# jaeyong-song/network_distributed_pytorch

Hardware: AMD Instinct MI355X
Metric: samples/sec + bytes/step all-reduced, ResNet18 CIFAR10 PowerSGD r=4, 1/2/4/8 GPU (higher is better)
Workload: dtype fp32; 1 GPU; model=resnet18, num_classes=1000, global_batch=512, per_gpu_batch=512, parallelism=dp1, reducer=powersgd, powersgd_rank=4, overlap=False, link_emulation=none, channels_last=False, stock_model_ops=False, hip_graph=full, tuned_gemms=True

## Files before the change

network_distributed_pytorch_amd/csrc/bindings.cpp:

```cpp
#include <algorithm>
#include <ATen/hip/HIPContext.h>
#include <torch/extension.h>

#include <cstring>

#include "ndp_kernels.h"
#include "plan.h"

namespace {

using ndp::MatGeom;
using ndp::MatPtrs;
using ndp::PItem;
using ndp::QItem;
using ndp::SegEntry;
using ndp::UItem;

hipStream_t cur_stream() { return at::hip::getCurrentHIPStream().stream(); }

void check_launch(const char* what) {
  const hipError_t err = hipGetLastError();
  TORCH_CHECK(err == hipSuccess, what, ": ", hipGetErrorString(err));
}

// ... 1060 lines not shown
  const int64_t M = g.size(0);
  const int N = (int)g.size(1);
  const int chunks = ndp::colsum_chunks(M, N);
  float* dp = deferred_part(part_out, (int64_t)chunks * N, "gelu_bwd_colsum");
  torch::Tensor part;
  if (dp == nullptr) part = torch::empty({(int64_t)chunks * N}, g.options());
  ndp::launch_gelu_bwd_colsum(g.data_ptr<float>(), h.data_ptr<float>(), dh.data_ptr<float>(), M, N,
                              dp ? dp : part.data_ptr<float>(), dp ? nullptr : db.data_ptr<float>(), cur_stream());
  check_launch("launch_gelu_bwd_colsum");
  return dp ? chunks : 0;
}

void ce_fwd(torch::Tensor x, torch::Tensor tgt, torch::Tensor dl, torch::Tensor scratch, torch::Tensor loss,
            torch::Tensor ctr, int64_t ignore_index, c10::optional<torch::Tensor> acc) {
  check_f32(x, "logits"); check_f32(dl, "dl"); check_f32(scratch, "scratch"); check_f32(loss, "loss");
  float* ap = nullptr;
  if (acc.has_value()) {
    check_f32(*acc, "acc");
    TORCH_CHECK(acc->numel() == 1, "ce_fwd: acc must be a one-element fp32 tensor");
    ap = acc->data_ptr<float>();
  }
  check_dev(tgt, "target"); check_dev(ctr, "ctr");
  TORCH_CHECK(x.dim() == 2 && x.is_contiguous() && dl.sizes() == x.sizes() && dl.is_contiguous(),
              "ce_fwd: logits / dl must be contiguous [B, K]");
  TORCH_CHECK(tgt.scalar_type() == torch::kInt64 && tgt.is_contiguous() && tgt.numel() == x.size(0),
              "ce_fwd: target must be contiguous int64 [B]");
  TORCH_CHECK(scratch.numel() >= x.size(0) + 1 && loss.numel() == 1, "ce_fwd: scratch / loss size");
  TORCH_CHECK(ctr.scalar_type() == torch::kInt32 && ctr.numel() >= 1, "ce_fwd: int32 counter");
  TORCH_CHECK(x.size(0) >= 1 && x.size(0) < (1LL << 31) && x.size(1) >= 1, "ce_fwd: empty batch");
  const int B = (int)x.size(0);
  float* sp = scratch.data_ptr<float>();
  ndp::launch_ce_fwd(x.data_ptr<float>(), tgt.data_ptr<int64_t>(), B, (int)x.size(1), ignore_index,
                     dl.data_ptr<float>(), sp, loss.data_ptr<float>(), sp + B,
                     reinterpret_cast<unsigned*>(ctr.data_ptr<int32_t>()), cur_stream(), ap);
  check_launch("launch_ce_fwd");
}

void ce_bwd(torch::Tensor dl, torch::Tensor g, torch::Tensor scratch, torch::Tensor dx) {
  check_f32(dl, "dl"); check_f32(g, "grad"); check_f32(scratch, "scratch"); check_f32(dx, "dx");
  TORCH_CHECK(dl.is_contiguous() && dx.is_contiguous() && dx.sizes() == dl.sizes() && dl.dim() == 2, "ce_bwd: shapes");
  TORCH_CHECK(g.numel() == 1 && scratch.numel() >= dl.size(0) + 1, "ce_bwd: scalar grad / scratch");
  TORCH_CHECK((reinterpret_cast<uintptr_t>(dl.data_ptr()) & 15) == 0 && (reinterpret_cast<uintptr_t>(dx.data_ptr()) & 15) == 0,
              "ce_bwd: 16-B aligned tensors");
  ndp::launch_ce_bwd(dl.data_ptr<float>(), g.data_ptr<float>(), scratch.data_ptr<float>() + dl.size(0),
                     dx.data_ptr<float>(), dl.numel(), cur_stream());
  check_launch("launch_ce_bwd");
}

static ndp::LnDrop ln_drop(int64_t mode, double p, const c10::optional<torch::Tensor>& seed,
                           const c10::optional<torch::Tensor>& da, int64_t numel) {
  ndp::LnDrop d{nullptr, 0u, 1.f, 0, nullptr};
  if (mode == 0 || p <= 0.0) return d;
  TORCH_CHECK(mode == 1 || mode == 2, "ln: dropout mode 0 / 1 / 2");
  TORCH_CHECK(p < 1.0, "ln: dropout p < 1");
  TORCH_CHECK(seed.has_value() && seed->is_cuda() && seed->scalar_type() == torch::kInt32 && seed->numel() >= 1,
              "ln: dropout needs a device int32 seed");
  d.seed = seed->data_ptr<int32_t>();
  const double t = p * 4294967296.0;
  d.thr = t >= 4294967295.0 ? 0xFFFFFFFFu : (uint32_t)t;
  d.scale = (float)(1.0 / (1.0 - p));
  d.mode = (int)mode;
  if (da.has_value()) {
    check_f32(*da, "da");
    TORCH_CHECK(da->is_contiguous() && da->numel() == numel, "ln: da [R, D]");
    d.da = da->data_ptr<float>();
  }
  return d;
}

void ln_fwd(torch::Tensor a, c10::optional<torch::Tensor> b, torch::Tensor gamma, torch::Tensor beta, torch::Tensor y,
            torch::Tensor s, torch::Tensor mean, torch::Tensor rstd, double eps, int64_t drop_mode, double p,
            c10::optional<torch::Tensor> seed) {
  check_f32(a, "a"); check_f32(gamma, "gamma"); check_f32(beta, "beta"); check_f32(y, "y"); check_f32(s, "s");
  check_f32(mean, "mean"); check_f32(rstd, "rstd");
  const int D = (int)a.size(-1);
  TORCH_CHECK(ndp::ln_supported(D) && gamma.numel() == D && beta.numel() == D, "ln_fwd: unsupported D");
  const int64_t R = a.numel() / D;
  for (auto* t : {&a, &y, &s}) TORCH_CHECK(t->is_contiguous() && t->numel() == R * D, "ln_fwd: contiguous [R, D]");
  if (b.has_value()) {
    check_f32(*b, "b");
    TORCH_CHECK(b->is_contiguous() && b->sizes() == a.sizes(), "ln_fwd: residual shape");
  }
  TORCH_CHECK(mean.numel() == R && rstd.numel() == R, "ln_fwd: stats size");
  ndp::launch_ln_fwd(a.data_ptr<float>(), opt_f32(b, "b"), gamma.data_ptr<float>(), beta.data_ptr<float>(),
                     y.data_ptr<float>(), s.data_ptr<float>(), mean.data_ptr<float>(), rstd.data_ptr<float>(), R, D,
                     (float)eps, cur_stream(), ln_drop(drop_mode, p, seed, c10::nullopt, R * D));
  check_launch("launch_ln_fwd");
}

int64_t ln_bwd(torch::Tensor dy, torch::Tensor s, torch::Tensor mean, torch::Tensor rstd, torch::Tensor gamma,
               torch::Tensor dx, torch::Tensor dgb, int64_t drop_mode, double p, c10::optional<torch::Tensor> seed,
               c10::optional<torch::Tensor> da, c10::optional<torch::Tensor> part_out) {
  check_f32(dy, "dy"); check_f32(s, "s"); check_f32(mean, "mean"); check_f32(rstd, "rstd"); check_f32(gamma, "gamma");
  check_f32(dx, "dx"); check_f32(dgb, "dgb");
  const int D = (int)s.size(-1);
  const int64_t R = s.numel() / D;
  TORCH_CHECK(ndp::ln_supported(D) && gamma.numel() == D && dgb.numel() == 2 * D, "ln_bwd: unsupported D");
  for (auto* t : {&dy, &s, &dx}) TORCH_CHECK(t->is_contiguous() && t->numel() == R * D, "ln_bwd: contiguous [R, D]");
  const ndp::LnDrop dp = ln_drop(drop_mode, p, seed, da, R * D);
  TORCH_CHECK(dp.mode != 1 || dp.da != nullptr, "ln_bwd: input dropout needs da");
  const int wgs = ndp::ln_bwd_wgs(R);
  float* pp = deferred_part(part_out, (int64_t)wgs * 2 * D, "ln_bwd");
  torch::Tensor part;
  if (pp == nullptr) part = torch::empty({(int64_t)wgs * 2 * D}, s.options());
  ndp::launch_ln_bwd(dy.data_ptr<float>(), s.data_ptr<float>(), mean.data_ptr<float>(), rstd.data_ptr<float>(),
                     gamma.data_ptr<float>(), dx.data_ptr<float>(), pp ? pp : part.data_ptr<float>(),
                     pp ? nullptr : dgb.data_ptr<float>(), R, D, cur_stream(), dp);
  check_launch("launch_ln_bwd");
  return pp ? wgs : 0;
}

void embedding_backward(torch::Tensor ids, torch::Tensor gout, torch::Tensor gw, int64_t pad, torch::Tensor perm,
                        torch::Tensor row_start, torch::Tensor row_cnt) {
  check_dev(ids, "ids"); check_f32(gout, "grad_out"); check_f32(gw, "grad_weight");
  check_dev(perm, "perm"); check_dev(row_start, "row_start"); check_dev(row_cnt, "row_cnt");
  TORCH_CHECK(ids.scalar_type() == torch::kInt64 && ids.is_contiguous(), "embedding_backward: ids must be contiguous int64");
  TORCH_CHECK(gw.dim() == 2 && gw.size(1) % 4 == 0, "embedding_backward: grad_weight [V, D] with D % 4 == 0");
  const int64_t T = ids.numel(), V = gw.size(0), D = gw.size(1);
  TORCH_CHECK(gout.numel() == T * D, "embedding_backward: grad_out must be [T, D]");
  TORCH_CHECK((reinterpret_cast<uintptr_t>(gout.data_ptr()) & 15) == 0 && (reinterpret_cast<uintptr_t>(gw.data_ptr()) & 15) == 0,
              "embedding_backward: 16-B aligned grad tensors");
  for (auto* t : {&perm, &row_start, &row_cnt})
    TORCH_CHECK(t->scalar_type() == torch::kInt32 && t->is_contiguous(), "embedding_backward: int32 scratch");
  TORCH_CHECK(perm.numel() >= T && row_start.numel() >= V && row_cnt.numel() >= V, "embedding_backward: scratch too small");
  TORCH_CHECK(T < (1LL << 29) && V < (1LL << 31), "embedding_backward: too many tokens / rows");
  ndp::launch_embedding_backward(ids.data_ptr<int64_t>(), (int)T, gout.data_ptr<float>(), (int)V, (int)D, (int)pad,
                                 perm.data_ptr<int32_t>(), row_start.data_ptr<int32_t>(), row_cnt.data_ptr<int32_t>(),
                                 gw.data_ptr<float>(), cur_stream());
  check_launch("launch_embedding_backward");
}

void attn_check(const torch::Tensor& t, const char* n, const torch::Tensor& q) {
  check_f32(t, n);
  TORCH_CHECK(t.sizes() == q.sizes() && t.is_contiguous(), n, ": contiguous [B, S, H, 64] like q");
}

int64_t attn_ld(const torch::Tensor& t, const char* n, const torch::Tensor& q) {
  TORCH_CHECK(t.is_cuda(), n, " must be a device (HIP) tensor");
  TORCH_CHECK(t.scalar_type() == torch::kFloat32 && t.sizes() == q.sizes(), n, ": fp32 [B, S, H, 64] like q");
  const int64_t S = t.size(1), H = t.size(2), ld = t.stride(1);
  TORCH_CHECK(t.stride(3) == 1 && t.stride(2) == 64 && t.stride(0) == S * ld && ld >= H * 64 && ld % 4 == 0 &&
                  (reinterpret_cast<uintptr_t>(t.data_ptr()) & 15) == 0,
              n, ": needs [B, S, H, 64] rows with a 16-B aligned token stride");
  return ld;
}

const int32_t* attn_seed(const c10::optional<torch::Tensor>& seed, double p_drop) {
  TORCH_CHECK(p_drop >= 0.0 && p_drop < 1.0, "attn: p_drop in [0, 1)");
  if (p_drop == 0.0) return nullptr;
  TORCH_CHECK(seed.has_value(), "attn: dropout needs a device seed tensor");
  check_dev(*seed, "seed");
  TORCH_CHECK(seed->scalar_type() == torch::kInt32 && seed->numel() >= 1, "attn: seed must be int32[1]");
  return seed->data_ptr<int32_t>();
}

void attn_fwd(torch::Tensor q, torch::Tensor k, torch::Tensor v, c10::optional<torch::Tensor> mask, torch::Tensor o,
              torch::Tensor lse, double scale, c10::optional<torch::Tensor> seed, double p_drop) {
  TORCH_CHECK(q.dim() == 4 && q.size(3) == 64, "attn: q must be [B, S, H, 64]");
  const int64_t ld = attn_ld(q, "q", q);
  TORCH_CHECK(attn_ld(k, "k", q) == ld && attn_ld(v, "v", q) == ld, "attn: q / k / v need one token stride");
  attn_check(o, "o", q); check_f32(lse, "lse");
  const int B = (int)q.size(0), S = (int)q.size(1), H = (int)q.size(2);
  TORCH_CHECK(lse.numel() >= 2 * (int64_t)B * H * S, "attn: lse must hold 2*B*H*S floats");
  const int32_t* mp = nullptr;
  if (mask.has_value()) {
    check_dev(*mask, "mask");
    TORCH_CHECK(mask->scalar_type() == torch::kInt32 && mask->is_contiguous() && mask->numel() == (int64_t)B * S,
                "attn: mask must be int32 [B, S]");
    mp = mask->data_ptr<int32_t>();
  }
  const int32_t* sp = attn_seed(seed, p_drop);
  ndp::launch_attn_fwd(q.data_ptr<float>(), k.data_ptr<float>(), v.data_ptr<float>(), mp, o.data_ptr<float>(),
                       lse.data_ptr<float>(), B, S, H, (float)scale, sp, (float)p_drop, cur_stream(), ld);
  check_launch("launch_attn_fwd");
}

void attn_bwd(torch::Tensor q, torch::Tensor k, torch::Tensor v, c10::optional<torch::Tensor> mask, torch::Tensor o,
              torch::Tensor dout, torch::Tensor lse, torch::Tensor delta, torch::Tensor dq, torch::Tensor dk,
              torch::Tensor dv, double scale, c10::optional<torch::Tensor> seed, double p_drop) {
  TORCH_CHECK(q.dim() == 4 && q.size(3) == 64, "attn: q must be [B, S, H, 64]");
  const int64_t ld = attn_ld(q, "q", q);
  for (auto* t : {&k, &v, &dq, &dk, &dv})
    TORCH_CHECK(attn_ld(*t, "q/k/v grads", q) == ld, "attn: q / k / v and their grads need one token stride");
  attn_check(o, "o", q); attn_check(dout, "dout", q);
  check_f32(lse, "lse"); check_f32(delta, "delta");
  const int B = (int)q.size(0), S = (int)q.size(1), H = (int)q.size(2);
  TORCH_CHECK(lse.numel() >= 2 * (int64_t)B * H * S && delta.numel() >= (int64_t)B * H * S,
              "attn: lse/delta too small");
  const int32_t* mp = nullptr;
  if (mask.has_value()) {
    check_dev(*mask, "mask");
    TORCH_CHECK(mask->scalar_type() == torch::kInt32 && mask->is_contiguous() && mask->numel() == (int64_t)B * S,
                "attn: mask must be int32 [B, S]");
    mp = mask->data_ptr<int32_t>();
  }
  const int32_t* sp = attn_seed(seed, p_drop);
  ndp::launch_attn_bwd(q.data_ptr<float>(), k.data_ptr<float>(), v.data_ptr<float>(), mp, o.data_ptr<float>(),
                       dout.data_ptr<float>(), lse.data_ptr<float>(), delta.data_ptr<float>(), dq.data_ptr<float>(),
                       dk.data_ptr<float>(), dv.data_ptr<float>(), B, S, H, (float)scale, sp,
                       (float)p_drop, cur_stream(), ld);
  check_launch("launch_attn_bwd");
}

}

void register_comm(py::module& m);
namespace ndp {
void* ipc_new(int rank, int nranks, int device, int64_t capacity_bytes);
void ipc_delete(void* c);
std::string ipc_handle(void* c);
void ipc_open(void* c, const std::vector<std::string>& h);
void ipc_all_reduce_many(void* c, const std::vector<at::Tensor>& ts, const std::string& op, int64_t stream);
int64_t ipc_error(void* c);
void ipc_check(void* c);
void ipc_destroy(void* c);
std::string ipc_bus_id(void* c);
int64_t ipc_info(void* c, int what);
}

struct IpcCommPy {
  void* c;
  IpcCommPy(int rank, int nranks, int device, int64_t cap) : c(ndp::ipc_new(rank, nranks, device, cap)) {}
  ~IpcCommPy() { ndp::ipc_delete(c); }
};

void register_ipc(py::module& m) {
  py::class_<IpcCommPy, std::shared_ptr<IpcCommPy>>(m, "IpcComm")
      .def(py::init<int, int, int, int64_t>(), py::arg("rank"), py::arg("nranks"), py::arg("device"),
           py::arg("capacity_bytes") = 8 << 20)
      .def("handle", [](IpcCommPy& s) { return py::bytes(ndp::ipc_handle(s.c)); })
      .def("open", [](IpcCommPy& s, const std::vector<std::string>& h) { ndp::ipc_open(s.c, h); })
      .def("all_reduce", [](IpcCommPy& s, torch::Tensor t, const std::string& op, int64_t stream) {
            ndp::ipc_all_reduce_many(s.c, {t}, op, stream);
          }, py::arg("t"), py::arg("op") = "sum", py::arg("stream") = 0)
      .def("all_reduce_many", [](IpcCommPy& s, const std::vector<torch::Tensor>& ts, const std::string& op,
                                 int64_t stream) { ndp::ipc_all_reduce_many(s.c, ts, op, stream); },
           py::arg("ts"), py::arg("op") = "sum", py::arg("stream") = 0)
      .def("error", [](IpcCommPy& s) { return ndp::ipc_error(s.c); })
      .def("check", [](IpcCommPy& s) { ndp::ipc_check(s.c); })
      .def("destroy", [](IpcCommPy& s) { ndp::ipc_destroy(s.c); })
      .def("bus_id", [](IpcCommPy& s) { return ndp::ipc_bus_id(s.c); })
      .def_property_readonly("rank", [](IpcCommPy& s) { return ndp::ipc_info(s.c, 0); })
      .def_property_readonly("nranks", [](IpcCommPy& s) { return ndp::ipc_info(s.c, 1); })
      .def_property_readonly("device", [](IpcCommPy& s) { return ndp::ipc_info(s.c, 2); })
      .def_property_readonly("capacity", [](IpcCommPy& s) { return ndp::ipc_info(s.c, 3); })
      .def_property_readonly("alive", [](IpcCommPy& s) { return ndp::ipc_info(s.c, 4) != 0; })
      .def_property_readonly("uncached", [](IpcCommPy& s) { return ndp::ipc_info(s.c, 5) != 0; })
      .def_property_readonly("launches", [](IpcCommPy& s) { return ndp::ipc_info(s.c, 6); });
}

PYBIND11_MODULE(TORCH_EXTENSION_NAME, m) {
  m.doc() = "network_distributed_pytorch_amd native gfx950 kernels + plan builder";
  m.attr("SIZEOF_MATGEOM") = (int)sizeof(MatGeom);
  m.attr("SIZEOF_MATPTRS") = (int)sizeof(MatPtrs);
  m.attr("SIZEOF_SEGENTRY") = (int)sizeof(SegEntry);
  m.attr("MAX_RANK") = ndp::kMaxRank;
  m.def("build_plan", &build_plan, "Build the PowerSGD execution plan (host)");
  m.def("patch_geom_vec", &patch_geom_vec);
  m.def("make_mat_ptrs", &make_mat_ptrs);
  m.def("make_seg_table", &make_seg_table);
  m.def("make_orth_geom", &make_orth_geom);
  m.def("psgd_p", &psgd_p, py::arg("geom"), py::arg("ptrs"), py::arg("items"), py::arg("q_warm"), py::arg("p_part"),
        py::arg("fuse_ef"), py::arg("max_rank"), py::arg("p_prev") = OptT(), py::arg("p_out") = OptT(),
        py::arg("p_ctr") = OptT(), py::arg("seg_entries") = OptT(), py::arg("seg_prefix") = OptT(),
        py::arg("seg_n") = 0, py::arg("seg_blocks") = 0, py::arg("p_cols") = (int64_t)ndp::kPKW);
  m.def("psgd_q", &psgd_q, py::arg("geom"), py::arg("ptrs"), py::arg("items"), py::arg("p_hat"), py::arg("q_part"),
        py::arg("max_rank"), py::arg("q_out") = OptT(), py::arg("q_ctr") = OptT(), py::arg("q_fin_max") = 1 << 30);
  m.def("psgd_orth", &psgd_orth, py::arg("geom"), py::arg("items"), py::arg("p"), py::arg("p_div"),
        py::arg("eps"), py::arg("max_rank"), py::arg("scratch"), py::arg("ctr"), py::arg("n_items_total") = -1,
        py::arg("max_spins") = -1);
  m.def("orth_coresident_cap", &ndp::orth_coresident_cap);
  m.def("psgd_update", &psgd_update, py::arg("geom"), py::arg("ptrs"), py::arg("items"), py::arg("p_hat"),
        py::arg("q_sum"), py::arg("q_div"), py::arg("q_warm"), py::arg("mode"), py::arg("lr"), py::arg("momentum"),
        py::arg("max_rank"), py::arg("p_prev") = c10::optional<torch::Tensor>(), py::arg("r1_buf") = OptT(),
        py::arg("r1_div") = 1.0, py::arg("r1_mom") = OptT(), py::arg("r1_x") = OptT(), py::arg("r1_g") = OptT());
  m.def("rank1_step", &rank1_step);
  m.def("seg_reduce", &seg_reduce);
  m.def("sgd_momentum", &sgd_momentum);
  m.def("add", &add);
  m.def("delay_ns", &delay_ns);
  m.def("bn_fwd", &bn_fwd, py::arg("x"), py::arg("res"), py::arg("y"), py::arg("gamma"), py::arg("beta"),
        py::arg("rmean"), py::arg("rvar"), py::arg("nbt"), py::arg("save_mean"), py::arg("save_invstd"),
        py::arg("part"), py::arg("eps"), py::arg("momentum"), py::arg("relu"), py::arg("training"),
        py::arg("single"), py::arg("xpart") = py::none(), py::arg("nslab") = 0, py::arg("xstats") = py::none(),
        py::arg("xS") = 0);
  m.def("bn_bwd", &bn_bwd, py::arg("dy"), py::arg("y"), py::arg("x"), py::arg("gamma"), py::arg("save_mean"),
        py::arg("save_invstd"), py::arg("dx"), py::arg("dres"), py::arg("dgamma"), py::arg("dbeta"), py::arg("part"),
        py::arg("relu"), py::arg("single"), py::arg("dypart") = py::none(), py::arg("nslab") = 0,
        py::arg("dyadd") = py::none(), py::arg("mbeta") = py::none(), py::arg("dstats") = py::none(),
        py::arg("dS") = 0);
  m.def("bn_relu_maxpool", &bn_relu_maxpool, py::arg("x"), py::arg("y"), py::arg("idx"), py::arg("gamma"),
        py::arg("beta"), py::arg("rmean"), py::arg("rvar"), py::arg("nbt"), py::arg("save_mean"),
        py::arg("save_invstd"), py::arg("part"), py::arg("eps"), py::arg("momentum"), py::arg("xstats") = py::none(),
        py::arg("xS") = 0);
  m.def("bn_two_kernel_path", [](int64_t N, int64_t C, int64_t HW, bool single) {
    return ndp::bn_two_kernel_path((int)N, (int)C, (int)HW, single ? 1 : 0);
  });
  m.def("bn_set_vec4", &ndp::bn_set_vec4);
  m.def("bn_pair_ok", &ndp::bn_pair_ok);
  m.def("bn_pair_fwd", &bn_pair_fwd);
  m.def("bn_pair_bwd", &bn_pair_bwd);
  m.def("wino_set_enabled", &ndp::wino_set_enabled);
  m.def("conv_set_stem_psplit", &ndp::conv_set_stem_psplit);
  m.def("bn_slices", &bn_slices);
  m.def("slab_sum", &slab_sum);
  m.def("bn_part_numel", &bn_part_numel);
  m.def("maxpool_fwd", &maxpool_fwd);
  m.def("maxpool_bwd", &maxpool_bwd);
  m.def("maxpool_bwd_bnstats", &maxpool_bwd_bnstats, py::arg("dy"), py::arg("idx"), py::arg("dx"), py::arg("x"),
        py::arg("gamma"), py::arg("beta"), py::arg("mean"), py::arg("invstd"), py::arg("stats"));
  m.def("stem_pool_bwd_apply", &stem_pool_bwd_apply);
  m.def("checksum", &checksum);
  m.def("flag_signal", &flag_signal);
  m.def("flag_wait", &flag_wait, py::arg("flags"), py::arg("i"), py::arg("seen"), py::arg("err"),
        py::arg("timeout_us"), py::arg("host_err") = c10::optional<torch::Tensor>());
  m.def("toeplitz_expand", &toeplitz_expand);
  m.def("toeplitz_fold", &toeplitz_fold);
  m.def("toeplitz_expand_many", &toeplitz_expand_many);
  m.def("toeplitz_fold_many", &toeplitz_fold_many);
  m.def("slab_sum_many", &slab_sum_many);
  m.def("gradw_finish", &gradw_finish, py::arg("slabs"), py::arg("folds"));
  m.def("conv_plan", &conv_plan, py::arg("geom"), py::arg("batch"));
  m.def("conv_fwd", &conv_fwd, py::arg("x"), py::arg("w"), py::arg("y"), py::arg("geom"), py::arg("part") = py::none(),
        py::arg("defer") = false, py::arg("stats") = py::none(), py::arg("wino_u") = py::none(),
        py::arg("pair") = false);
  m.def("conv_flush_pending_fwd", []() {
    ndp::conv_flush_pending_fwd();
    check_launch("conv_flush_pending_fwd");
  });
  m.def("wino_weights", &wino_weights);
  m.def("wino_weights_many", &wino_weights_many);
  m.def("conv_wino", [](const std::vector<int64_t>& geom, int64_t B, bool dgrad) {
    const ndp::ConvGeom g = conv_geom(geom);
    const int cls = ndp::conv_direct_class(g);
    return cls >= 0 && B > 0 && B % ndp::conv_fwd_imgs(cls) == 0 && ndp::conv_wino(cls, g, (int)B, dgrad);
  });
  m.def("conv_stats_slices", &conv_stats_slices, py::arg("geom"), py::arg("batch"));
  m.def("conv_dgrad", &conv_dgrad, py::arg("dy"), py::arg("w"), py::arg("dx"), py::arg("geom"),
        py::arg("part") = py::none(), py::arg("addend") = py::none(), py::arg("defer") = false,
        py::arg("stats") = py::none(), py::arg("bn_x") = py::none(), py::arg("bn_y") = py::none(),
        py::arg("bn_mean") = py::none(), py::arg("bn_invstd") = py::none(), py::arg("wino_u") = py::none());
  m.def("conv_dgrad_stats_slices", [](const std::vector<int64_t>& geom, int64_t B) -> int64_t {
    const ndp::ConvGeom g = conv_geom(geom);
    const int cls = ndp::conv_direct_class(g);
    if (cls < 0 || B <= 0 || B % ndp::conv_fwd_imgs(cls)) return 0;
    return ndp::conv_dgrad_stats_slices(cls, g, (int)B);
  }, py::arg("geom"), py::arg("batch"));
  m.def("conv_wgrad", &conv_wgrad, py::arg("x"), py::arg("dy"), py::arg("part"), py::arg("dw"), py::arg("geom"),
        py::arg("pair") = false);
  m.def("conv_flush_pending", []() {
    ndp::conv_flush_pending();
    check_launch("conv_flush_pending");
  });
  m.def("tg_plan", &tg_plan);
  m.def("tg_describe", &tg_describe);
  m.def("tg_fwd", &tg_fwd, py::arg("x"), py::arg("w"), py::arg("y"), py::arg("geom"), py::arg("part") = py::none(),
        py::arg("defer") = false);
  m.def("tg_dgrad", &tg_dgrad, py::arg("dy"), py::arg("w"), py::arg("dx"), py::arg("geom"),
        py::arg("part") = py::none(), py::arg("addend") = py::none(), py::arg("defer") = false);
  m.def("tg_wgrad", &tg_wgrad, py::arg("x"), py::arg("dy"), py::arg("out"), py::arg("geom"),
        py::arg("part") = py::none(), py::arg("defer") = false);
  m.def("embedding_backward", &embedding_backward);
  m.def("colsum", &colsum, py::arg("g"), py::arg("out"), py::arg("part") = c10::optional<torch::Tensor>());
  m.def("gelu_bwd_colsum", &gelu_bwd_colsum, py::arg("g"), py::arg("h"), py::arg("dh"), py::arg("db"),
        py::arg("part") = c10::optional<torch::Tensor>());
  m.def("ce_fwd", &ce_fwd, py::arg("x"), py::arg("tgt"), py::arg("dl"), py::arg("scratch"), py::arg("loss"),
        py::arg("ctr"), py::arg("ignore_index"), py::arg("acc") = py::none());
  m.def("ln_fwd", &ln_fwd, py::arg("a"), py::arg("b"), py::arg("gamma"), py::arg("beta"), py::arg("y"), py::arg("s"),
        py::arg("mean"), py::arg("rstd"), py::arg("eps"), py::arg("drop_mode") = 0, py::arg("p") = 0.0,
        py::arg("seed") = c10::optional<torch::Tensor>());
  m.def("ln_bwd", &ln_bwd, py::arg("dy"), py::arg("s"), py::arg("mean"), py::arg("rstd"), py::arg("gamma"),
        py::arg("dx"), py::arg("dgb"), py::arg("drop_mode") = 0, py::arg("p") = 0.0,
        py::arg("seed") = c10::optional<torch::Tensor>(), py::arg("da") = c10::optional<torch::Tensor>(),
        py::arg("part") = c10::optional<torch::Tensor>());
  m.def("ln_bwd_wgs", [](int64_t R) { return (int64_t)ndp::ln_bwd_wgs(R); });
  m.def("colsum_chunks", [](int64_t M, int64_t N) { return (int64_t)ndp::colsum_chunks(M, (int)N); });
  m.def("ce_bwd", &ce_bwd);
  m.def("attn_fwd", &attn_fwd);
  m.def("attn_bwd", &attn_bwd);
  register_comm(m);
  register_ipc(m);
}
```

network_distributed_pytorch_amd/csrc/conv.hip:

```cpp
#include <hip/hip_runtime.h>
#include <stdlib.h>

#include "ndp_kernels.h"
#include "wino_dpp.h"

namespace ndp {

typedef float f32x4e __attribute__((ext_vector_type(4)));

__global__ __launch_bounds__(256) void toeplitz_expand_kernel(const float* __restrict__ w, float* __restrict__ wt,
                                                              ConvGeom g) {
  const int K = g.C * g.H * g.W;
  const int kcol = blockIdx.x * 256 + threadIdx.x;
  if (kcol >= K) return;
  const int n = blockIdx.y;
  const int OHW = g.OH * g.OW;
  const int co = n / OHW, ohw = n - co * OHW;
  const int oh = ohw / g.OW, ow = ohw - oh * g.OW;
  const int HW = g.H * g.W;
  const int ci = kcol / HW, ihw = kcol - ci * HW;
  const int ih = ihw / g.W, iw = ihw - ih * g.W;
  const int kh = ih - oh * g.stride + g.pad, kw = iw - ow * g.stride + g.pad;
  float v = 0.f;
  if (kh >= 0 && kh < g.KH && kw >= 0 && kw < g.KW) v = w[((co * g.C + ci) * g.KH + kh) * g.KW + kw];
  wt[(int64_t)n * K + kcol] = v;
}

template <int H, int W>
__device__ __forceinline__ void expand_row(const float* __restrict__ w, float* __restrict__ row, const ConvGeom& g,
                                           int co, int oh, int ow) {
  const int h0 = oh * g.stride - g.pad, w0 = ow * g.stride - g.pad;
  for (int ci = threadIdx.x; ci < g.C; ci += 256) {
    const float* wc = w + ((int64_t)co * g.C + ci) * g.KH * g.KW;
    float v[H * W];
#pragma unroll
    for (int ih = 0; ih < H; ++ih)
#pragma unroll
      for (int iw = 0; iw < W; ++iw) {
        const int kh = ih - h0, kw = iw - w0;
        v[ih * W + iw] = (kh >= 0 && kh < g.KH && kw >= 0 && kw < g.KW) ? wc[kh * g.KW + kw] : 0.f;
      }
    float* d = row + (int64_t)ci * (H * W);
    if constexpr ((H * W) % 4 == 0) {
#pragma unroll
      for (int j = 0; j < H * W; j += 4)
        *reinterpret_cast<f32x4e*>(d + j) = f32x4e{v[j], v[j + 1], v[j + 2], v[j + 3]};
    } else {
#pragma unroll
      for (int j = 0; j < H * W; ++j) d[j] = v[j];
    }
  }
}

__global__ __launch_bounds__(256) void toeplitz_expand_many_kernel(ExpandBatch b) {
  const int64_t r = blockIdx.x;
  int e = 0;
  while (e + 1 < b.n && r >= b.end[e]) ++e;
  const ConvGeom& g = b.g[e];
  const int n = (int)(r - (e ? b.end[e - 1] : 0));
  const int OHW = g.OH * g.OW;
  const int co = n / OHW, ohw = n - co * OHW;
  const int oh = ohw / g.OW, ow = ohw - oh * g.OW;
  float* row = b.wt[e] + (int64_t)n * g.C * g.H * g.W;
  if (g.H == 1 && g.W == 1) expand_row<1, 1>(b.w[e], row, g, co, oh, ow);
  else if (g.H == 2 && g.W == 2) expand_row<2, 2>(b.w[e], row, g, co, oh, ow);
  else if (g.H == 4 && g.W == 4) expand_row<4, 4>(b.w[e], row, g, co, oh, ow);
  else {
    const int K = g.C * g.H * g.W, HW = g.H * g.W;
    for (int kcol = threadIdx.x; kcol < K; kcol += 256) {
      const int ci = kcol / HW, ihw = kcol - ci * HW;
      const int ih = ihw / g.W, iw = ihw - ih * g.W;
      const int kh = ih - oh * g.stride + g.pad, kw = iw - ow * g.stride + g.pad;
      float v = 0.f;
      if (kh >= 0 && kh < g.KH && kw >= 0 && kw < g.KW) v = b.w[e][((co * g.C + ci) * g.KH + kh) * g.KW + kw];
      row[kcol] = v;
    }
  }
}

constexpr int kExpandRows = 8;
template <int H, int W>
__device__ __forceinline__ void expand_rows(const float* __restrict__ w, float* __restrict__ wt, const ConvGeom& g,
                                            int n0) {
  const int C = g.C, OHW = g.OH * g.OW;
  const int64_t K = (int64_t)C * H * W;
  for (int idx = threadIdx.x; idx < kExpandRows * C; idx += 256) {
    const int rr = idx / C, ci = idx - rr * C;
    const int n = n0 + rr;
    const int co = n / OHW, ohw = n - co * OHW;
    const int oh = ohw / g.OW, ow = ohw - oh * g.OW;
    const int h0 = oh * g.stride - g.pad, w0 = ow * g.stride - g.pad;
    const float* wc = w + ((int64_t)co * C + ci) * g.KH * g.KW;
    float v[H * W];
#pragma unroll
    for (int ih = 0; ih < H; ++ih)
#pragma unroll
      for (int iw = 0; iw < W; ++iw) {
        const int kh = ih - h0, kw = iw - w0;
        v[ih * W + iw] = (kh >= 0 && kh < g.KH && kw >= 0 && kw < g.KW) ? wc[kh * g.KW + kw] : 0.f;
      }
    float* d = wt + (int64_t)n * K + (int64_t)ci * (H * W);
    if constexpr ((H * W) % 4 == 0) {
#pragma unroll
      for (int j = 0; j < H * W; j += 4)
        *reinterpret_cast<f32x4e*>(d + j) = f32x4e{v[j], v[j + 1], v[j + 2], v[j + 3]};
    } else {
#pragma unroll
      for (int j = 0; j < H * W; ++j) d[j] = v[j];
    }
  }
}

__global__ __launch_bounds__(256) void toeplitz_expand_rows_kernel(ExpandBatch b) {
  const int64_t r0 = (int64_t)blockIdx.x * kExpandRows;
  int e = 0;
  while (e + 1 < b.n && r0 >= b.end[e]) ++e;
  const ConvGeom& g = b.g[e];
  const int n0 = (int)(r0 - (e ? b.end[e - 1] : 0));
  if (g.H == 1 && g.W == 1) expand_rows<1, 1>(b.w[e], b.wt[e], g, n0);
  else if (g.H == 2 && g.W == 2) expand_rows<2, 2>(b.w[e], b.wt[e], g, n0);
  else expand_rows<4, 4>(b.w[e], b.wt[e], g, n0);
}

void launch_toeplitz_expand_many(const ExpandBatch& b, hipStream_t s) {
  if (b.n <= 0) return;
  bool rows_ok = true;
  for (int e = 0; e < b.n; ++e) {
    const ConvGeom& g = b.g[e];
    const int64_t rows = b.end[e] - (e ? b.end[e - 1] : 0);
    rows_ok = rows_ok && rows % kExpandRows == 0 && g.H == g.W && (g.H == 1 || g.H == 2 || g.H == 4);
  }
  if (rows_ok)
    hipLaunchKernelGGL(toeplitz_expand_rows_kernel, dim3((unsigned)(b.end[b.n - 1] / kExpandRows)), dim3(256), 0, s,
                       b);
  else
    hipLaunchKernelGGL(toeplitz_expand_many_kernel, dim3((unsigned)b.end[b.n - 1]), dim3(256), 0, s, b);
}

constexpr int kFoldMaxTaps = 9;
__device__ __forceinline__ void fold_pair(const float* __restrict__ dwt, const ConvGeom& g, int pair,
                                          float (&acc)[kFoldMaxTaps]) {
  const int co = pair / g.C, ci = pair - co * g.C;
  const int K = g.C * g.H * g.W, HW = g.H * g.W;
#pragma unroll
  for (int t = 0; t < kFoldMaxTaps; ++t) acc[t] = 0.f;
  for (int oh = 0; oh < g.OH; ++oh)
    for (int ow = 0; ow < g.OW; ++ow) {
      const float* row = dwt + (int64_t)((co * g.OH + oh) * g.OW + ow) * K + ci * HW;
      for (int ih = 0; ih < g.H; ++ih) {
        const int kh = ih - oh * g.stride + g.pad;
        if (kh < 0 || kh >= g.KH) continue;
        for (int iw = 0; iw < g.W; ++iw) {
          const int kw = iw - ow * g.stride + g.pad;
          if (kw < 0 || kw >= g.KW) continue;
          const float v = row[ih * g.W + iw];
#pragma unroll
          for (int t = 0; t < kFoldMaxTaps; ++t)
            if (t == kh * g.KW + kw) acc[t] += v;
        }
      }
    }
}

template <int H, int W, int OH, int OW, int ST, int PD, int KH, int KW>
__device__ __forceinline__ void fold_pair_t(const float* __restrict__ dwt, int C, int pair,
                                            float (&acc)[kFoldMaxTaps]) {
  const int co = pair / C, ci = pair - co * C;
  const int64_t K = (int64_t)C * H * W;
#pragma unroll
  for (int t = 0; t < kFoldMaxTaps; ++t) acc[t] = 0.f;
  float v[OH * OW][H * W];
#pragma unroll
  for (int oh = 0; oh < OH; ++oh)
#pragma unroll
    for (int ow = 0; ow < OW; ++ow) {
      const float* row = dwt + (int64_t)((co * OH + oh) * OW + ow) * K + (int64_t)ci * (H * W);
#pragma unroll
      for (int ih = 0; ih < H; ++ih)
#pragma unroll
        for (int iw = 0; iw < W; ++iw) {
          const int kh = ih - oh * ST + PD, kw = iw - ow * ST + PD;
          v[oh * OW + ow][ih * W + iw] = (kh >= 0 && kh < KH && kw >= 0 && kw < KW) ? row[ih * W + iw] : 0.f;
        }
    }
#pragma unroll
  for (int oh = 0; oh < OH; ++oh)
#pragma unroll
    for (int ow = 0; ow < OW; ++ow)
#pragma unroll
      for (int ih = 0; ih < H; ++ih)
#pragma unroll
        for (int iw = 0; iw < W; ++iw) {
          const int kh = ih - oh * ST + PD, kw = iw - ow * ST + PD;
          if (kh >= 0 && kh < KH && kw >= 0 && kw < KW) acc[kh * KW + kw] += v[oh * OW + ow][ih * W + iw];
        }
}

__device__ __forceinline__ void fold_any(const float* __restrict__ dwt, const ConvGeom& g, int pair,
                                         float (&acc)[kFoldMaxTaps]) {
  const bool k3 = g.KH == 3 && g.KW == 3 && g.pad == 1, k1 = g.KH == 1 && g.KW == 1 && g.pad == 0;
  if (k3 && g.H == 2 && g.W == 2 && g.stride == 1) fold_pair_t<2, 2, 2, 2, 1, 1, 3, 3>(dwt, g.C, pair, acc);
  else if (k3 && g.H == 4 && g.W == 4 && g.stride == 2) fold_pair_t<4, 4, 2, 2, 2, 1, 3, 3>(dwt, g.C, pair, acc);
  else if (k1 && g.H == 4 && g.W == 4 && g.stride == 2) fold_pair_t<4, 4, 2, 2, 2, 0, 1, 1>(dwt, g.C, pair, acc);
  else if (k3 && g.H == 2 && g.W == 2 && g.stride == 2) fold_pair_t<2, 2, 1, 1, 2, 1, 3, 3>(dwt, g.C, pair, acc);
  else if (k1 && g.H == 2 && g.W == 2 && g.stride == 2) fold_pair_t<2, 2, 1, 1, 2, 0, 1, 1>(dwt, g.C, pair, acc);
  else if (k3 && g.H == 1 && g.W == 1 && g.stride == 1) fold_pair_t<1, 1, 1, 1, 1, 1, 3, 3>(dwt, g.C, pair, acc);
  else fold_pair(dwt, g, pair, acc);
}

__device__ __forceinline__ void fold_many_block(const FoldBatch& b, int64_t blk, float* __restrict__ stage) {
  const int64_t base = blk * 256;
  const int64_t i = base + threadIdx.x;
  const int64_t total = b.end[b.n - 1];
  int e = 0;
  while (e + 1 < b.n && base >= b.end[e]) ++e;
  const int64_t e_lo = e ? b.end[e - 1] : 0;
  const bool one_entry = base + 256 <= b.end[e];
  if (one_entry) {
    const ConvGeom& g = b.g[e];
    const int T = g.KH * g.KW;
    float acc[kFoldMaxTaps];
    fold_any(b.dwt[e], g, (int)(i - e_lo), acc);
#pragma unroll
    for (int t = 0; t < kFoldMaxTaps; ++t)
      if (t < T) stage[threadIdx.x * T + t] = acc[t];
    __syncthreads();
    float* out = b.dw[e] + (base - e_lo) * T;
    for (int k = threadIdx.x; k < 256 * T; k += 256) out[k] = stage[k];
    return;
  }
  if (i >= total) return;
  while (e + 1 < b.n && i >= b.end[e]) ++e;
  const ConvGeom& g = b.g[e];
  const int T = g.KH * g.KW;
  const int pair = (int)(i - (e ? b.end[e - 1] : 0));
  float acc[kFoldMaxTaps];
  fold_any(b.dwt[e], g, pair, acc);
  float* out = b.dw[e] + (int64_t)pair * T;
#pragma unroll
  for (int t = 0; t < kFoldMaxTaps; ++t)
    if (t < T) out[t] = acc[t];
}

__global__ __launch_bounds__(256) void toeplitz_fold_many_kernel(FoldBatch b) {
  __shared__ float stage[256 * kFoldMaxTaps];
  fold_many_block(b, blockIdx.x, stage);
}

void launch_toeplitz_fold_many(const FoldBatch& b, hipStream_t s) {
  if (b.n <= 0) return;
  const int64_t total = b.end[b.n - 1];
  hipLaunchKernelGGL(toeplitz_fold_many_kernel, dim3((unsigned)((total + 255) / 256)), dim3(256), 0, s, b);
}

void launch_toeplitz_expand(const float* w, float* wb, const ConvGeom& g, hipStream_t s) {
  const int N = g.Co * g.OH * g.OW, K = g.C * g.H * g.W;
  hipLaunchKernelGGL(toeplitz_expand_kernel, dim3((K + 255) / 256, N), dim3(256), 0, s, w, wb, g);
}

void launch_toeplitz_fold(const float* dwb, float* dw, const ConvGeom& g, hipStream_t s) {
  FoldBatch b{};
  b.dwt[0] = dwb;
  b.dw[0] = dw;
  b.g[0] = g;
  b.end[0] = (int64_t)g.Co * g.C;
  b.n = 1;
  launch_toeplitz_fold_many(b, s);
}



typedef float f32x16 __attribute__((ext_vector_type(16)));
typedef float f32x4c __attribute__((ext_vector_type(4)));

__device__ __forceinline__ f32x16 mfma32(float a, float b, f32x16 c) {
  return __builtin_amdgcn_mfma_f32_32x32x2f32(a, b, c, 0, 0, 0);
}

template <int R, int S, int ST, int PD, int H, int W, int CK, int BM, int IMGS, int WM, int NBUF, int KB, bool TRANSW,
          int PSPLIT = 1>
struct ConvFwdCfg {
  static constexpr int P = (H + 2 * PD - R) / ST + 1, Q = (W + 2 * PD - S) / ST + 1, PQ = P * Q;
  static_assert(PSPLIT == 1 || (IMGS == 1 && P % PSPLIT == 0), "row blocks of one image");
  static constexpr int LAYOUT = (ST == 1 && H == 8 && W == 8 && PD == 1 && IMGS == 1) ? 1
                                : (ST == 1 && H == 4 && W == 4 && IMGS % 2 == 0)      ? 2
                                : (ST == 2 && H == 8 && W == 8 && IMGS % 2 == 0)      ? 3
                                : (ST == 2 && H == 32 && W == 32 && R == 7 && IMGS == 1) ? 4
                                                                                       : 0;
  static constexpr bool DEINT = LAYOUT == 4;
  static constexpr int HALF = (W + 2 * PD + 2) / 2;
  static constexpr int Hp = H + 2 * PD;
  static constexpr int Wp = LAYOUT == 1 ? 12 : LAYOUT == 2 ? 8 : LAYOUT == 3 ? 12 : DEINT ? 2 * HALF : W + 2 * PD;
  __device__ static __forceinline__ constexpr int cpos(int col) {
    return DEINT ? (col & 1) * HALF + (col >> 1) : col;
  }
  static constexpr int HWp = (Hp * Wp) | 1, HW = H * W;
  static constexpr int IPAD0 = LAYOUT == 2 ? 4 : LAYOUT == 3 ? 1 : 0;
  static constexpr int IMGSTR = LAYOUT >= 2 ? (CK * HWp + 31) / 32 * 32 + IPAD0 : CK * HWp;
  static_assert(Wp >= W + 2 * PD && (!DEINT || (ST == 2 && HALF * 2 == Wp && (ST * Wp) % 32 == 16)),
                "row stride holds the zero border");
  __device__ static __forceinline__ void pix(int n, int& img, int& p, int& q) {
    if constexpr (LAYOUT == 1) {
      img = 0;
      p = (n & 31) >> 2;
// ... 145 lines not shown
      if (e < AE) {
        if (VEC) {
          if (!TRANSW) {
            const int r = e >> 2, k4 = r % (G::KK / 4), m = 4 * (r / (G::KK / 4)) + (e & 3);
            if constexpr (G::AV) {
              *reinterpret_cast<f32x4c*>(A + m * G::LDAM + 4 * k4) = ra[i];
            } else {
              float* d = A + 4 * k4 * G::LDA + m;
              d[0] = ra[i].x; d[G::LDA] = ra[i].y; d[2 * G::LDA] = ra[i].z; d[3 * G::LDA] = ra[i].w;
            }
          } else {
            const int c = e / (BM * G::RS / 4), f = 4 * (e - c * (BM * G::RS / 4));
#pragma unroll
            for (int j = 0; j < 4; ++j) {
              const int m = (f + j) / G::RS, rs = (f + j) - m * G::RS;
              const int kk = c * G::RS + (G::RS - 1 - rs);
              if constexpr (G::AV) A[m * G::LDAM + kk] = ra[i][j];
              else A[kk * G::LDA + m] = ra[i][j];
            }
          }
        } else {
#pragma unroll
          for (int j = 0; j < 4; ++j) {
            const int f = 4 * e + j, m = f / G::KK, kk = f - m * G::KK;
            if (f < BM * G::KK) {
              if constexpr (G::PAIRK) {
                const int row = G::pk_row(kk);
                if (row >= 0) A[row * G::LDA + m] = ra[i][j];
              } else if constexpr (G::AV) {
                A[m * G::LDAM + kk] = ra[i][j];
              } else {
                A[kk * G::LDA + m] = ra[i][j];
              }
            }
          }
        }
      }
    }
#pragma unroll
    for (int i = 0; i < BPT; ++i) {
      const int e = tid + 256 * i;
      if (e < B4I) {
        const int img = e / (CK * IHW / 4), rem = 4 * (e - img * (CK * IHW / 4));
        const int c = rem / IHW, hw = rem - c * IHW;
        const int hh = hw / IW, ww = hw - hh * IW;
        if constexpr (G::DEINT) {
          float* d = B + img * G::IMGSTR + c * G::HWp + (hh + PD) * G::Wp;
#pragma unroll
          for (int j = 0; j < 4; ++j) d[G::cpos(ww + PD + j)] = rb[i][j];
        } else {
          float* d = B + img * G::IMGSTR + c * G::HWp + (IUPS * hh + PD) * G::Wp + IUPS * ww + PD;
          d[0] = rb[i].x; d[IUPS] = rb[i].y; d[2 * IUPS] = rb[i].z; d[3 * IUPS] = rb[i].w;
        }
      }
    }
  };

  f32x16 acc[G::TM][G::TN];
#pragma unroll
  for (int tm = 0; tm < G::TM; ++tm)
#pragma unroll
    for (int tn = 0; tn < G::TN; ++tn)
#pragma unroll
      for (int r = 0; r < 16; ++r) acc[tm][tn][r] = 0.f;

  load(0);
  __syncthreads();
  store(0);
  __syncthreads();
  for (int ch = 0; ch < nchunks; ++ch) {
    const int cur = (NBUF == 2) ? (ch & 1) : 0;
    if (NBUF == 2 && ch + 1 < nchunks) load(ch + 1);
    const float* A = As + cur * G::A_SZ;
    const float* B = Bs + cur * G::B_SZ;
    float av[2][KB][G::TM], bv[2][KB][G::TN];
    auto fetch = [&](int blk, int slot) {
#pragma unroll
      for (int i = 0; i < KB; ++i) {
        const int t = blk * KB + i;
        int c = t / G::RS, rs = t - c * G::RS, r = rs / S, s = rs - r * S;
        if constexpr (G::PAIRK) {
          c = G::pk_c(t);
          r = G::pk_r(t);
          s = G::pk_s(t);
        }
        const int offb = c * G::HWp + r * G::Wp + (G::DEINT ? (s & 1) * G::HALF + (s >> 1) : s);
        if constexpr (!G::AV) {
#pragma unroll
          for (int tm = 0; tm < G::TM; ++tm) av[slot][i][tm] = A[a_base[tm] + t * G::LDA];
        }
#pragma unroll
        for (int tn = 0; tn < G::TN; ++tn) {
          if constexpr (G::PAIRK) bv[slot][i][tn] = B[(t < 56 ? b_base[tn] : b_base2[tn]) + offb];
          else bv[slot][i][tn] = B[b_base[tn] + offb];
        }
      }
      if constexpr (G::AV) {
#pragma unroll
        for (int tm = 0; tm < G::TM; ++tm)
#pragma unroll
          for (int q = 0; q < KB / 4; ++q) {
            const f32x4c v = *reinterpret_cast<const f32x4c*>(A + a_base[tm] + blk * KB + 4 * q);
#pragma unroll
            for (int j = 0; j < 4; ++j) av[slot][4 * q + j][tm] = v[j];
          }
      }
    };
    if constexpr (SCH == 1) __builtin_amdgcn_iglp_opt(0);
    fetch(0, 0);
#pragma unroll
    for (int blk = 0; blk < G::NBLK; ++blk) {
      if (blk + 1 < G::NBLK) fetch(blk + 1, (blk + 1) & 1);
#pragma unroll
      for (int i = 0; i < KB; ++i)
#pragma unroll
        for (int tm = 0; tm < G::TM; ++tm)
#pragma unroll
          for (int tn = 0; tn < G::TN; ++tn)
            acc[tm][tn] = mfma32(av[blk & 1][i][tm], bv[blk & 1][i][tn], acc[tm][tn]);
    }
    if constexpr (SCH == 2) {
#pragma unroll
      for (int i = 0; i < G::NSTEP * G::TM * G::TN; ++i) {
        __builtin_amdgcn_sched_group_barrier(0x008, 1, 0);
        __builtin_amdgcn_sched_group_barrier(0x100, 1, 0);
      }
    }
    if (ch + 1 < nchunks) {
      if (NBUF == 2) {
        store(cur ^ 1);
      } else {
        __syncthreads();
        load(ch + 1);
        store(0);
      }
    }
    __syncthreads();
  }

  if (gdim.z > 1) {
    float* pz = part + (int64_t)bid.z * slab;
#pragma unroll
    for (int tm = 0; tm < G::TM; ++tm)
#pragma unroll
      for (int tn = 0; tn < G::TN; ++tn) {
        const int n = (wn * G::TN + tn) * 32 + l32;
        int img, p, q;
        G::pix(n, img, p, q);
        p += prow0;
        float* pb = pz + (int64_t)(b0 + img) * Kout * G::PQ + p * G::Q + q;
#pragma unroll
        for (int r = 0; r < 16; ++r) {
          const int m = m0 + (wm * G::TM + tm) * 32 + (r & 3) + 8 * (r >> 2) + 4 * h;
          pb[(int64_t)m * G::PQ] = acc[tm][tn][r];
        }
      }
    return;
  }

  constexpr int OPQ = G::PQ * UPS * UPS;
  constexpr bool kStats = G::STATS_OK && UPS == 1;
  const bool stats = kStats && st.out != nullptr;
  const bool bstats = G::STATS2_OK && stats && st.bx != nullptr;
  float* L = smem;
  float* L2 = smem + BM * G::STATS_LDO;
#pragma unroll
  for (int tm = 0; tm < G::TM; ++tm)
#pragma unroll
    for (int tn = 0; tn < G::TN; ++tn) {
      const int n = (wn * G::TN + tn) * 32 + l32;
      int img, pp, qq;
      G::pix(n, img, pp, qq);
      pp += prow0;
      const int opix = UPS == 1 ? pp * G::Q + qq : pp * UPS * (UPS * G::Q) + qq * UPS;
      const int64_t yoff = (int64_t)(b0 + img) * Kout * OPQ + opix;
      float* yb = y + yoff;
      float ad[16], ad1[UPS == 2 ? 16 : 1], ad2[UPS == 2 ? 16 : 1], ad3[UPS == 2 ? 16 : 1];
      if (addend != nullptr) {
#pragma unroll
        for (int r = 0; r < 16; ++r) {
          const int m = m0 + (wm * G::TM + tm) * 32 + (r & 3) + 8 * (r >> 2) + 4 * h;
          const float* ap = addend + yoff + (int64_t)m * OPQ;
          ad[r] = ap[0];
          if constexpr (UPS == 2) {
            ad1[r] = ap[1];
            ad2[r] = ap[2 * G::Q];
            ad3[r] = ap[2 * G::Q + 1];
          }
        }
      } else {
#pragma unroll
        for (int r = 0; r < 16; ++r) {
          ad[r] = 0.f;
          if constexpr (UPS == 2) ad1[r] = ad2[r] = ad3[r] = 0.f;
        }
      }
      float bxv[16], byv[16], bmu[16], bis[16];
      if (kStats && bstats) {
#pragma unroll
        for (int r = 0; r < 16; ++r) {
          const int m = m0 + (wm * G::TM + tm) * 32 + (r & 3) + 8 * (r >> 2) + 4 * h;
          bxv[r] = st.bx[yoff + (int64_t)m * OPQ];
          byv[r] = st.by[yoff + (int64_t)m * OPQ];
          bmu[r] = st.mean[m];
          bis[r] = st.invstd[m];
        }
      }
#pragma unroll
      for (int r = 0; r < 16; ++r) {
        const int mloc = (wm * G::TM + tm) * 32 + (r & 3) + 8 * (r >> 2) + 4 * h;
        const int m = m0 + mloc;
        float* d = yb + (int64_t)m * OPQ;
        const float v = acc[tm][tn][r] + ad[r];
        d[0] = v;
        if constexpr (UPS == 2) {
          d[1] = ad1[r];
          d[2 * G::Q] = ad2[r];
          d[2 * G::Q + 1] = ad3[r];
        }
        if constexpr (kStats) {
          if (bstats) {
            const float dz = byv[r] > 0.f ? v : 0.f;
            L[mloc * G::STATS_LDO + n] = dz;
            L2[mloc * G::STATS_LDO + n] = dz * ((bxv[r] - bmu[r]) * bis[r]);
          } else if (stats) {
            L[mloc * G::STATS_LDO + n] = v;
          }
        }
      }
    }

  if constexpr (kStats) {
    if (stats) {
      __syncthreads();
      constexpr int TPC = G::STATS_TPC, NPT = G::BN / TPC;
      const int c = tid / TPC, j = tid - c * TPC;
      const float* src = L + c * G::STATS_LDO + j * NPT;
      const float* src2 = L2 + c * G::STATS_LDO + j * NPT;
      double sum = 0.0, sq = 0.0;
#pragma unroll 4
      for (int i = 0; i < NPT; i += 4) {
        const f32x4c v = *reinterpret_cast<const f32x4c*>(src + i);
        sum += (double)((v.x + v.y) + (v.z + v.w));
        if (bstats) {
          const f32x4c u = *reinterpret_cast<const f32x4c*>(src2 + i);
          sq += (double)((u.x + u.y) + (u.z + u.w));
        } else {
          sq += (double)((v.x * v.x + v.y * v.y) + (v.z * v.z + v.w * v.w));
        }
      }
#pragma unroll
      for (int o = 1; o < TPC; o <<= 1) {
        sum += __shfl_xor(sum, o, 64);
        sq += __shfl_xor(sq, o, 64);
      }
      if (j == 0) {
        double* d = st.out + ((int64_t)(m0 + c) * gdim.x + bid.x) * 2;
        d[0] = sum;
        d[1] = sq;
      }
    }
  }
}

template <int R, int S, int ST, int PD, int H, int W, int CK, int BM, int IMGS, int WM, int NBUF, int KB, bool TRANSW,
          bool VEC, int UPS = 1, int SCH = 0, int IUPS = 1, int PSPLIT = 1>
__global__ __launch_bounds__(256) void conv_fwd_kernel(const float* __restrict__ x, const float* __restrict__ w,
                                                       float* __restrict__ y, float* __restrict__ part, int Cin,
                                                       int Kout, int cps, int64_t slab,
                                                       const float* __restrict__ addend, ConvBnStats st) {
  extern __shared__ __attribute__((aligned(16))) float smem[];
  conv_fwd_body<R, S, ST, PD, H, W, CK, BM, IMGS, WM, NBUF, KB, TRANSW, VEC, UPS, SCH, IUPS, PSPLIT>(
      x, w, y, part, Cin, Kout, cps, slab, addend, st, make_uint3(blockIdx.x, blockIdx.y, blockIdx.z),
      make_uint3(gridDim.x, gridDim.y, gridDim.z), smem);
}

template <int R, int S, int ST, int PD, int H, int W, int CB, int BM, int NW, int NBPW, int KB>
struct ConvWgCfg {
  static constexpr int P = (H + 2 * PD - R) / ST + 1, Q = (W + 2 * PD - S) / ST + 1, PQ = P * Q;
  static constexpr int Hp = H + 2 * PD, Wp = W + 2 * PD, HWp = (Hp * Wp) | 1, HW = H * W;
  static constexpr int RS = R * S, J = CB * RS, JB = (J + 31) / 32, MB = BM / 32;
  static constexpr bool TAPMAJ = CB % 32 == 0;
  __device__ static __forceinline__ void col(int j, int& c, int& rs) {
    if constexpr (TAPMAJ) {
      rs = j / CB;
      c = j - rs * CB;
    } else {
      c = j / RS;
      rs = j - c * RS;
    }
  }
  static constexpr int NSTEP = PQ / 2, NBLK = NSTEP / KB;
  static constexpr bool AVW = KB % 4 == 0 && (PQ / 2) % 4 == 0;
  static constexpr int LDY = AVW ? PQ + (((PQ / 4) % 2 == 0) ? 4 : 8) : PQ + 1;
  static constexpr int A_SZ = BM * LDY;
  static constexpr int B_SZ = CB * HWp;
  static constexpr int NT = 64 * NW;
  static constexpr int A4 = BM * PQ / 4, B4 = CB * HW / 4;
  static constexpr int A_PER_T = (A4 + NT - 1) / NT, B_PER_T = (B4 + NT - 1) / NT;
  static constexpr int LDJ = J + 4;
  static constexpr size_t MAIN_BYTES = 2 * (size_t)(A_SZ + B_SZ) * sizeof(float);
  static constexpr size_t EPI_BYTES = TAPMAJ ? (size_t)BM * LDJ * sizeof(float) : 0;
  static constexpr size_t LDS_BYTES = MAIN_BYTES > EPI_BYTES ? MAIN_BYTES : EPI_BYTES;
  static_assert(MB * JB == NW * NBPW, "every wave owns NBPW 32x32 blocks");
  static_assert(P % 2 == 0 && PQ % 4 == 0 && HW % 4 == 0 && NSTEP % KB == 0, "pixel pairing / float4 loads");
};

template <int R, int S, int ST, int PD, int H, int W, int CB, int BM, int NW, int NBPW, int KB>
__device__ __forceinline__ void conv_wgrad_body(const float* __restrict__ x, const float* __restrict__ dy,
                                                float* __restrict__ part, int Cin, int Kout, int imgs_per_slice,
                                                const uint3 bid, float* __restrict__ smem) {
  using G = ConvWgCfg<R, S, ST, PD, H, W, CB, BM, NW, NBPW, KB>;
  float* As = smem;
  float* Bs = smem + 2 * G::A_SZ;
  const int tid = threadIdx.x, lane = tid & 63, wave = tid >> 6;
  const int h = lane >> 5, l32 = lane & 31;
  const int slice = bid.x, m0 = bid.y * BM, c0 = bid.z * CB;
  const int bb = slice * imgs_per_slice;

  for (int i = tid; i < 2 * G::B_SZ; i += G::NT) Bs[i] = 0.f;

  int a_base[NBPW], b_base[NBPW];
#pragma unroll
  for (int t = 0; t < NBPW; ++t) {
    const int blk = wave * NBPW + t;
    const int mb = blk / G::JB, jb = blk - mb * G::JB;
    const int j = jb * 32 + l32;
    a_base[t] = (mb * 32 + l32) * G::LDY + h * (G::PQ / 2);
    int c, rs;
    G::col(j, c, rs);
    const int r = rs / S, s = rs - r * S;
    b_base[t] = (j < G::J) ? c * G::HWp + r * G::Wp + s + h * (G::P / 2) * ST * G::Wp : 0;
  }

  f32x4c ra[G::A_PER_T], rb[G::B_PER_T];
  auto load = [&](int b) {
#pragma unroll
    for (int i = 0; i < G::A_PER_T; ++i) {
      const int e = tid + G::NT * i;
      f32x4c v = {0.f, 0.f, 0.f, 0.f};
      if (e < G::A4) v = *reinterpret_cast<const f32x4c*>(dy + ((int64_t)b * Kout + m0) * G::PQ + 4 * e);
      ra[i] = v;
    }
#pragma unroll
    for (int i = 0; i < G::B_PER_T; ++i) {
      const int e = tid + G::NT * i;
      f32x4c v = {0.f, 0.f, 0.f, 0.f};
      if (e < G::B4 && c0 + (4 * e) / G::HW < Cin)
        v = *reinterpret_cast<const f32x4c*>(x + ((int64_t)b * Cin + c0) * G::HW + 4 * e);
      rb[i] = v;
    }
  };
  auto store = [&](int buf) {
    float* A = As + buf * G::A_SZ;
    float* B = Bs + buf * G::B_SZ;
#pragma unroll
    for (int i = 0; i < G::A_PER_T; ++i) {
      const int e = tid + G::NT * i;
      if (e < G::A4) {
        const int m = (4 * e) / G::PQ, pq = 4 * e - m * G::PQ;
        float* d = A + m * G::LDY + pq;
        if constexpr (G::AVW) {
          *reinterpret_cast<f32x4c*>(d) = ra[i];
        } else {
          d[0] = ra[i].x; d[1] = ra[i].y; d[2] = ra[i].z; d[3] = ra[i].w;
        }
      }
    }
#pragma unroll
    for (int i = 0; i < G::B_PER_T; ++i) {
      const int e = tid + G::NT * i;
      if (e < G::B4) {
        const int c = (4 * e) / G::HW, hw = 4 * e - c * G::HW;
        const int hh = hw / W, ww = hw - hh * W;
        float* d = B + c * G::HWp + (hh + PD) * G::Wp + ww + PD;
        d[0] = rb[i].x; d[1] = rb[i].y; d[2] = rb[i].z; d[3] = rb[i].w;
      }
    }
  };

  f32x16 acc[NBPW];
#pragma unroll
  for (int t = 0; t < NBPW; ++t)
#pragma unroll
    for (int r = 0; r < 16; ++r) acc[t][r] = 0.f;

  load(bb);
  __syncthreads();
  store(0);
  __syncthreads();
  for (int i = 0; i < imgs_per_slice; ++i) {
    const int cur = i & 1;
    if (i + 1 < imgs_per_slice) load(bb + i + 1);
    const float* A = As + cur * G::A_SZ;
    const float* B = Bs + cur * G::B_SZ;
    float av[2][KB][NBPW], bv[2][KB][NBPW];
    auto fetch = [&](int blk, int slot) {
#pragma unroll
      for (int k = 0; k < KB; ++k) {
        const int t = blk * KB + k;
        const int p = t / G::Q, q = t - p * G::Q;
#pragma unroll
        for (int u = 0; u < NBPW; ++u) {
          if constexpr (!G::AVW) av[slot][k][u] = A[a_base[u] + t];
          bv[slot][k][u] = B[b_base[u] + p * ST * G::Wp + q * ST];
        }
      }
      if constexpr (G::AVW) {
#pragma unroll
        for (int u = 0; u < NBPW; ++u)
#pragma unroll
          for (int q4 = 0; q4 < KB / 4; ++q4) {
            const f32x4c v = *reinterpret_cast<const f32x4c*>(A + a_base[u] + blk * KB + 4 * q4);
#pragma unroll
            for (int j = 0; j < 4; ++j) av[slot][4 * q4 + j][u] = v[j];
          }
      }
    };
    fetch(0, 0);
#pragma unroll
    for (int blk = 0; blk < G::NBLK; ++blk) {
      if (blk + 1 < G::NBLK) fetch(blk + 1, (blk + 1) & 1);
#pragma unroll
      for (int k = 0; k < KB; ++k)
#pragma unroll
        for (int u = 0; u < NBPW; ++u) acc[u] = mfma32(av[blk & 1][k][u], bv[blk & 1][k][u], acc[u]);
    }
    if (i + 1 < imgs_per_slice) store(cur ^ 1);
    __syncthreads();
  }

  float* out = part + (int64_t)slice * Kout * Cin * G::RS;
  if constexpr (G::TAPMAJ && G::RS > 1) {
    float* st = smem;
#pragma unroll
    for (int t = 0; t < NBPW; ++t) {
      const int blk = wave * NBPW + t;
      const int mb = blk / G::JB, jb = blk - mb * G::JB;
      const int j = jb * 32 + l32;
      int c, rs;
      G::col(j, c, rs);
      if (j < G::J) {
#pragma unroll
        for (int r = 0; r < 16; ++r)
          st[(mb * 32 + (r & 3) + 8 * (r >> 2) + 4 * h) * G::LDJ + c * G::RS + rs] = acc[t][r];
      }
    }
    __syncthreads();
    const int lim = min(CB, Cin - c0) * G::RS;
    constexpr int J4 = G::J / 4;
    static_assert(G::J % 4 == 0, "float4 rows");
    for (int i = tid; i < BM * J4; i += G::NT) {
      const int mr = i / J4, q = 4 * (i - mr * J4);
      const f32x4c v = *reinterpret_cast<const f32x4c*>(st + mr * G::LDJ + q);
      float* o = out + ((int64_t)(m0 + mr) * Cin + c0) * G::RS + q;
      if (q + 3 < lim) {
        *reinterpret_cast<f32x4c*>(o) = v;
      } else {
#pragma unroll
        for (int k = 0; k < 4; ++k)
          if (q + k < lim) o[k] = v[k];
      }
    }
    return;
  }
#pragma unroll
  for (int t = 0; t < NBPW; ++t) {
    const int blk = wave * NBPW + t;
    const int mb = blk / G::JB, jb = blk - mb * G::JB;
    const int j = jb * 32 + l32;
    int c, rs;
    G::col(j, c, rs);
    if (j < G::J && c0 + c < Cin) {
#pragma unroll
      for (int r = 0; r < 16; ++r) {
        const int m = m0 + mb * 32 + (r & 3) + 8 * (r >> 2) + 4 * h;
        out[((int64_t)m * Cin + c0 + c) * G::RS + rs] = acc[t][r];
      }
    }
  }
}

template <int R, int S, int ST, int PD, int H, int W, int CB, int BM, int NW, int NBPW, int KB>
__global__ __launch_bounds__(64 * NW) void conv_wgrad_kernel(const float* __restrict__ x, const float* __restrict__ dy,
                                                             float* __restrict__ part, int Cin, int Kout,
                                                             int imgs_per_slice) {
  extern __shared__ __attribute__((aligned(16))) float smem[];
  conv_wgrad_body<R, S, ST, PD, H, W, CB, BM, NW, NBPW, KB>(x, dy, part, Cin, Kout, imgs_per_slice,
                                                           make_uint3(blockIdx.x, blockIdx.y, blockIdx.z), smem);
}

template <int WH, int IUPS, int R, int S, int ST, int PD, int H, int W, int CB, int BM, int NW, int NBPW, int KB>
__global__ __launch_bounds__(256, 2) void wino_direct_pair_kernel(WinoConvArgs A, uint3 ga, const float* __restrict__ x,
                                                                  const float* __restrict__ dy, float* __restrict__ part,
                                                                  int Cin, int Kout, int imgs, uint3 gw) {
  static_assert(NW <= 4, "grad-W workgroup within the pair's 256 threads");
  extern __shared__ __attribute__((aligned(16))) float smem[];
  const unsigned na = ga.x * ga.y * ga.z;
  unsigned b = blockIdx.x;
  if (b < na) {
    wino_dpp_body<WH, IUPS>(A, make_uint3(b % ga.x, (b / ga.x) % ga.y, b / (ga.x * ga.y)), ga, smem);
  } else {
    if (threadIdx.x >= 64 * NW) return;
    b -= na;
    conv_wgrad_body<R, S, ST, PD, H, W, CB, BM, NW, NBPW, KB>(
        x, dy, part, Cin, Kout, imgs, make_uint3(b % gw.x, (b / gw.x) % gw.y, b / (gw.x * gw.y)), smem);
  }
}

__global__ __launch_bounds__(256) void conv_slab_sum_kernel(const float* __restrict__ part, float* __restrict__ dw,
                                                            int64_t n, int n_slices,
                                                            const float* __restrict__ addend = nullptr) {
  __shared__ f32x4c red[16][16];
  const int col = threadIdx.x & 15, g = threadIdx.x >> 4;
  const int64_t i4 = ((int64_t)blockIdx.x * 16 + col) * 4;
  f32x4c acc = {0.f, 0.f, 0.f, 0.f};
  if (i4 < n) {
#pragma unroll 4
    for (int s = g; s < n_slices; s += 16) acc += *reinterpret_cast<const f32x4c*>(part + (int64_t)s * n + i4);
  }
  red[g][col] = acc;
  __syncthreads();
  if (g == 0 && i4 < n) {
    f32x4c t = red[0][col];
#pragma unroll
    for (int k = 1; k < 16; ++k) t += red[k][col];
    if (addend) t += *reinterpret_cast<const f32x4c*>(addend + i4);
    *reinterpret_cast<f32x4c*>(dw + i4) = t;
  }
}

__device__ __forceinline__ void slab_sum_many_block(const SlabBatch& b, int64_t blk, f32x4c (*red)[16]) {
  int e = 0;
  while (e + 1 < b.n && blk >= b.end[e]) ++e;
  const int64_t lb = blk - (e ? b.end[e - 1] : 0);
  const float* part = b.part[e];
  const int64_t n = b.numel[e];
  const int n_slices = b.slices[e];
  const int col = threadIdx.x & 15, g = threadIdx.x >> 4;
  const int64_t i4 = (lb * 16 + col) * 4;
  f32x4c acc = {0.f, 0.f, 0.f, 0.f};
  if (i4 < n) {
#pragma unroll 4
    for (int sl = g; sl < n_slices; sl += 16) {
      if (b.nt) acc += __builtin_nontemporal_load(reinterpret_cast<const f32x4c*>(part + (int64_t)sl * n + i4));
      else acc += *reinterpret_cast<const f32x4c*>(part + (int64_t)sl * n + i4);
    }
  }
  red[g][col] = acc;
  __syncthreads();
  if (g == 0 && i4 < n) {
    f32x4c t = red[0][col];
#pragma unroll
    for (int k = 1; k < 16; ++k) t += red[k][col];
    *reinterpret_cast<f32x4c*>(b.dw[e] + i4) = t;
  }
}

__global__ __launch_bounds__(256) void conv_slab_sum_many_kernel(SlabBatch b) {
  __shared__ f32x4c red[16][16];
  slab_sum_many_block(b, blockIdx.x, red);
}

__global__ __launch_bounds__(256) void gradw_finish_kernel(SlabBatch sb, FoldBatch fb) {
  constexpr int kFloats = 256 * kFoldMaxTaps > 16 * 16 * 4 ? 256 * kFoldMaxTaps : 16 * 16 * 4;
  __shared__ __attribute__((aligned(16))) float smem[kFloats];
  const int64_t n_slab = sb.n > 0 ? sb.end[sb.n - 1] : 0;
  const int64_t blk = blockIdx.x;
  if (blk < n_slab) slab_sum_many_block(sb, blk, reinterpret_cast<f32x4c (*)[16]>(smem));
  else fold_many_block(fb, blk - n_slab, smem);
}

void launch_gradw_finish(const SlabBatch& sb, const FoldBatch& fb, hipStream_t s) {
  if (sb.n <= 0) return launch_toeplitz_fold_many(fb, s);
  if (fb.n <= 0) return launch_slab_sum_many(sb, s);
  const_cast<SlabBatch&>(sb).nt = 1;
  const int64_t blocks = sb.end[sb.n - 1] + (fb.end[fb.n - 1] + 255) / 256;
  hipLaunchKernelGGL(gradw_finish_kernel, dim3((unsigned)blocks), dim3(256), 0, s, sb, fb);
}

void launch_slab_sum_many(const SlabBatch& b, hipStream_t s) {
  const_cast<SlabBatch&>(b).nt = 1;
  if (b.n <= 0) return;
  hipLaunchKernelGGL(conv_slab_sum_many_kernel, dim3((unsigned)b.end[b.n - 1]), dim3(256), 0, s, b);
}

template <int P, int Q>
__global__ __launch_bounds__(256) void conv_slab_sum_ups_kernel(const float* __restrict__ part, float* __restrict__ dx,
                                                                int64_t slab, int n_slices,
                                                                const float* __restrict__ addend) {
  constexpr int F4R = (2 * Q) / 4, F4P = 2 * P * F4R;
  static_assert((2 * Q) % 4 == 0, "float4 rows");
  const int64_t i4 = (int64_t)blockIdx.x * 256 + threadIdx.x;
  if (i4 * 4 >= slab * 4) return;
  const int64_t plane = i4 / F4P;
  const int r4 = (int)(i4 - plane * F4P);
  const int row = r4 / F4R, half = r4 - row * F4R;
  f32x4c v = {0.f, 0.f, 0.f, 0.f};
  if (addend != nullptr) v = *reinterpret_cast<const f32x4c*>(addend + i4 * 4);
  if ((row & 1) == 0) {
    const int p = row >> 1, q0 = half * 2;
    const float* src = part + plane * (P * Q) + p * Q + q0;
    float a = 0.f, b = 0.f;
    for (int z = 0; z < n_slices; ++z) {
      a += src[z * slab];
      b += src[z * slab + 1];
    }
    v.x += a;
    v.z += b;
  }
  *reinterpret_cast<f32x4c*>(dx + i4 * 4) = v;
}

template <typename KernelT>
static void set_lds(KernelT k, size_t bytes) {
  hipFuncSetAttribute(reinterpret_cast<const void*>(k), hipFuncAttributeMaxDynamicSharedMemorySize, (int)bytes);
}

struct DirectDgradArgs {
  const float* dy;
  const float* w;
  float* dx;
  float* part;
  int Cin, Kout, cps;
  int64_t slab;
  const float* addend;
};
template <int DH, int DW, int DBM, int DIMGS, int R, int S, int ST, int PD, int H, int W, int CB, int BM, int NW,
          int NBPW, int KB>
__global__ __launch_bounds__(256) void direct_pair_kernel(DirectDgradArgs A, uint3 ga, const float* __restrict__ x,
                                                          const float* __restrict__ dy, float* __restrict__ part,
                                                          int Cin, int Kout, int imgs, uint3 gw) {
  static_assert(NW <= 4, "grad-W workgroup within the pair's 256 threads");
  extern __shared__ __attribute__((aligned(16))) float smem[];
  const unsigned na = ga.x * ga.y * ga.z;
  unsigned b = blockIdx.x;
  if (b < na) {
    conv_fwd_body<1, 1, 1, 0, DH, DW, 8, DBM, DIMGS, 2, 2, 4, true, true, 2>(
        A.dy, A.w, A.dx, A.part, A.Cin, A.Kout, A.cps, A.slab, A.addend, ConvBnStats{},
        make_uint3(b % ga.x, (b / ga.x) % ga.y, b / (ga.x * ga.y)), ga, smem);
  } else {
    if (threadIdx.x >= 64 * NW) return;
    b -= na;
    conv_wgrad_body<R, S, ST, PD, H, W, CB, BM, NW, NBPW, KB>(
        x, dy, part, Cin, Kout, imgs, make_uint3(b % gw.x, (b / gw.x) % gw.y, b / (gw.x * gw.y)), smem);
  }
}

template <int R, int S, int ST, int PD, int H, int W, int CK, int BM, int IMGS, int WM, int NBUF, int KB, bool TRANSW,
          bool VEC, int UPS = 1, int SCH = 0, int IUPS = 1, int PSPLIT = 1>
static int run_fwd(const float* x, const float* w, float* y, int B, int Cin, int Kout, int ksplit, float* part,
                   hipStream_t s, const float* addend = nullptr, bool defer = false,
                   ConvBnStats stats = ConvBnStats{nullptr, nullptr, nullptr, nullptr, nullptr}) {
  using G = ConvFwdCfg<R, S, ST, PD, H, W, CK, BM, IMGS, WM, NBUF, KB, TRANSW, PSPLIT>;
  auto k = conv_fwd_kernel<R, S, ST, PD, H, W, CK, BM, IMGS, WM, NBUF, KB, TRANSW, VEC, UPS, SCH, IUPS, PSPLIT>;
  static bool attr = false;
  if (!attr) { set_lds(k, G::LDS_BYTES); attr = true; }
  const int nchunks = (Cin + CK - 1) / CK;
  if (ksplit < 1 || part == nullptr) ksplit = 1;
  const int cps = (nchunks + ksplit - 1) / ksplit;
  ksplit = (nchunks + cps - 1) / cps;
  const int64_t slab = (int64_t)B * Kout * G::PQ;
  if (!(G::STATS_OK && UPS == 1) || ksplit > 1 || (stats.bx != nullptr && !G::STATS2_OK)) stats.out = nullptr;
  hipLaunchKernelGGL(k, dim3(B / IMGS * PSPLIT, Kout / BM, ksplit), dim3(256), G::LDS_BYTES, s, x, w, y, part, Cin, Kout, cps,
                     slab, ksplit > 1 ? nullptr : addend, stats);
  if (ksplit > 1 && defer && UPS == 1) return ksplit;
  if (ksplit > 1) {
    if constexpr (UPS == 1)
      hipLaunchKernelGGL(conv_slab_sum_kernel, dim3((unsigned)((slab / 4 + 15) / 16)), dim3(256), 0, s, part, y, slab,
                         ksplit, addend);
    else
      hipLaunchKernelGGL((conv_slab_sum_ups_kernel<G::P, G::Q>), dim3((unsigned)((slab + 255) / 256)), dim3(256), 0, s,
                         part, y, slab, ksplit, addend);
  }
  return 1;
}

struct FwdPart {
  const float* x;
  const float* w;
  float* y;
  float* part;
  int Cin, Kout, cps;
  int64_t slab;
};
__global__ __launch_bounds__(256) void ds_fwd_pair_kernel(FwdPart a, uint3 ga, FwdPart b, uint3 gb) {
  extern __shared__ __attribute__((aligned(16))) float smem[];
  const unsigned na = ga.x * ga.y * ga.z;
  unsigned k = blockIdx.x;
  if (k < na) {
    conv_fwd_body<3, 3, 2, 1, 8, 8, 8, 64, 4, 2, 2, 4, false, true>(
        a.x, a.w, a.y, a.part, a.Cin, a.Kout, a.cps, a.slab, nullptr, ConvBnStats{},
        make_uint3(k % ga.x, (k / ga.x) % ga.y, k / (ga.x * ga.y)), ga, smem);
  } else {
    k -= na;
    conv_fwd_body<1, 1, 2, 0, 8, 8, 8, 64, 4, 2, 2, 4, false, true>(
        b.x, b.w, b.y, b.part, b.Cin, b.Kout, b.cps, b.slab, nullptr, ConvBnStats{},
        make_uint3(k % gb.x, (k / gb.x) % gb.y, k / (gb.x * gb.y)), gb, smem);
  }
}

template <typename G>
static FwdPart fwd_part(const float* x, const float* w, float* y, float* part, int B, int Cin, int Kout, int& ksplit) {
  const int nchunks = (Cin + 8 - 1) / 8;
  if (ksplit < 1 || part == nullptr) ksplit = 1;
  const int cps = (nchunks + ksplit - 1) / ksplit;
  ksplit = (nchunks + cps - 1) / cps;
  return FwdPart{x, w, y, part, Cin, Kout, cps, (int64_t)B * Kout * G::PQ};
}

void launch_slab_sum(const float* part, float* out, int64_t n, int nslab, hipStream_t s, const float* addend) {
  hipLaunchKernelGGL(conv_slab_sum_kernel, dim3((unsigned)((n / 4 + 15) / 16)), dim3(256), 0, s, part, out, n, nslab,
                     addend);
}

template <int R, int S, int ST, int PD, int H, int W, int CB, int BM, int NW, int NBPW, int KB>
static void run_wgrad(const float* x, const float* dy, float* part, float* dw, int B, int Cin, int Kout,
                      int imgs, hipStream_t s) {
  using G = ConvWgCfg<R, S, ST, PD, H, W, CB, BM, NW, NBPW, KB>;
  auto k = conv_wgrad_kernel<R, S, ST, PD, H, W, CB, BM, NW, NBPW, KB>;
  static bool attr = false;
  if (!attr) { set_lds(k, G::LDS_BYTES); attr = true; }
  const int slices = B / imgs;
  hipLaunchKernelGGL(k, dim3(slices, Kout / BM, (Cin + CB - 1) / CB), dim3(G::NT), G::LDS_BYTES, s, x, dy, part, Cin,
                     Kout, imgs);
  if (dw == nullptr) return;
  const int64_t n = (int64_t)Kout * Cin * G::RS;
  hipLaunchKernelGGL(conv_slab_sum_kernel, dim3((unsigned)((n / 4 + 15) / 16)), dim3(256), 0, s, part, dw, n, slices);
}

int conv_direct_class(const ConvGeom& g) {
  if (g.KH == 3 && g.KW == 3 && g.pad == 1 && g.stride == 1 && g.H == 8 && g.W == 8 && g.C % 64 == 0 && g.Co % 64 == 0)
    return 0;
  if (g.KH == 3 && g.KW == 3 && g.pad == 1 && g.stride == 1 && g.H == 4 && g.W == 4 && g.C % 64 == 0 && g.Co % 64 == 0)
    return 1;
  if (g.KH == 3 && g.KW == 3 && g.pad == 1 && g.stride == 2 && g.H == 8 && g.W == 8 && g.C % 64 == 0 && g.Co % 64 == 0)
    return 2;
  if (g.KH == 7 && g.KW == 7 && g.pad == 3 && g.stride == 2 && g.H == 32 && g.W == 32 && g.C == 3 && g.Co % 64 == 0)
    return 3;
  if (g.KH == 1 && g.KW == 1 && g.pad == 0 && g.stride == 2 && g.H == 8 && g.W == 8 && g.C % 64 == 0 && g.Co % 64 == 0)
    return 4;
  if (g.KH == 1 && g.KW == 1 && g.pad == 0 && g.stride == 2 && g.H == 4 && g.W == 4 && g.C % 64 == 0 && g.Co % 64 == 0)
    return 5;
  return -1;
}

int conv_fwd_imgs(int cls) { return (cls == 0 || cls == 3) ? 1 : cls == 5 ? 16 : 4; }

static constexpr int kFillWgs = 256;

static int pow2_floor(int v) {
  int p = 1;
  while (p * 2 <= v) p *= 2;
  return p;
}

int conv_wgrad_imgs(int cls, const ConvGeom& g, int B) {
  if (cls == 0 && g.H == 8 && g.C % 16 == 0 && g.Co % 16 == 0 && B <= 128 && B % 4 == 0) {
    const int per_slice = (g.Co / 16) * (g.C / 16);
    int d = 32;
    while (d > 4 && (B % d != 0 || (B / d) * per_slice < kFillWgs)) d /= 2;
    if (B % d == 0 && wino_wgrad_red(B, d)) return d;
  }
  if (cls == 0 && g.H == 8 && g.C % 16 == 0 && g.Co % 16 == 0 && B >= 256 && B % 16 == 0 && wino_wgrad_red(B, 16)) {
    return 16;
  }
  int def = cls == 0 ? 8 : cls == 1 ? (B >= 512 ? 32 : 16) : cls == 2 ? 16 : cls == 4 ? 8 : cls == 5 ? 16 : 4;
  const int cb = cls == 3 ? 3 : 32;
  const int per_slice = (g.Co / 32) * ((g.C + cb - 1) / cb);
  while (def > 1 && B % def != 0) def /= 2;
  while (def > 1 && (B / def) * per_slice < kFillWgs && B % (def / 2) == 0) def /= 2;
  return def;
}

static constexpr int kConvMaxSplit = 4;

int conv_ksplit(int cls, const ConvGeom& g, int B, bool dgrad) {
  if (cls < 0 || cls == 3) return 1;
  if (dgrad && (cls == 4 || cls == 5) && B >= 512) return 1;
  const int inC = dgrad ? g.Co : g.C, outC = dgrad ? g.C : g.Co;
  const int imgs = (dgrad && cls == 2) ? 1 : conv_fwd_imgs(cls);
  const int base = (B / imgs) * (outC / 64);
  const int nchunks = inC / 8;
  int ks = 1;
  while (ks * 2 <= nchunks && base * ks < kFillWgs && ks * 2 <= kConvMaxSplit) ks *= 2;
  return pow2_floor(ks);
}
static int wino_slabs(const float* part, float* out, int64_t n, int ks, bool defer, const float* addend,
                      hipStream_t s) {
  if (defer) return ks;
  hipLaunchKernelGGL(conv_slab_sum_kernel, dim3((unsigned)((n / 4 + 15) / 16)), dim3(256), 0, s, part, out, n, ks,
                     addend);
  return 1;
}

bool conv_wino(int cls, const ConvGeom& g, int B, bool dgrad) {
  if (dgrad)
    return (cls == 0 || cls == 1 || cls == 2) && wino_ok(g.Co, g.C, B, g.H, g.W, conv_ksplit(cls, g, B, true));
  return (cls == 0 || cls == 1) && wino_ok(g.C, g.Co, B, g.H, g.W, conv_ksplit(cls, g, B, false));
}

static int g_stem_psplit = 0;
void conv_set_stem_psplit(int p) { g_stem_psplit = (p == 1 || p == 2 || p == 4) ? p : 0; }
int stem_psplit(int B) {
  if (g_stem_psplit) return g_stem_psplit;
  return B >= 256 ? 1 : B >= 128 ? 2 : 4;
}

int conv_fwd_stats_slices(int cls, const ConvGeom& g, int B) {
  static_assert(ConvFwdCfg<3, 3, 1, 1, 8, 8, 8, 64, 1, 2, 2, 4, false>::STATS_OK &&
                    ConvFwdCfg<7, 7, 2, 3, 32, 32, 4, 64, 1, 2, 1, 7, false>::STATS_OK &&
                    ConvFwdCfg<7, 7, 2, 3, 32, 32, 4, 64, 1, 2, 1, 7, false, 2>::STATS_OK &&
                    ConvFwdCfg<7, 7, 2, 3, 32, 32, 4, 64, 1, 2, 1, 7, false, 4>::STATS_OK,
                "statistics epilogue fits every layer1 / stem tile");
  if (cls != 0 && cls != 3) return 0;
  if (conv_ksplit(cls, g, B, false) != 1) return 0;
  if (cls == 3) return B * stem_psplit(B);
  return conv_wino(cls, g, B, false) ? B / wino_imgs(g.H) : B / conv_fwd_imgs(cls);
}
int conv_dgrad_stats_slices(int cls, const ConvGeom& g, int B) {
  static_assert(ConvFwdCfg<3, 3, 1, 1, 8, 8, 8, 64, 1, 2, 2, 4, true>::STATS2_OK,
                "backward statistics epilogue fits the layer1 grad-x tiles");
  if ((cls != 0 && cls != 2) || conv_ksplit(cls, g, B, true) != 1) return 0;
  if (conv_wino(cls, g, B, true)) return B / wino_imgs(g.H);
  return cls == 2 ? B : B / conv_fwd_imgs(cls);
}
bool conv_dgrad_direct(int cls) { return cls >= 0 && cls <= 5 && cls != 3; }

namespace {
struct PendingFwd {
  const float* x = nullptr;
  const float* w = nullptr;
  float* y = nullptr;
  float* part = nullptr;
  int B = 0, ks = 1;
  bool defer = false;
  ConvGeom g{};
  hipStream_t s = nullptr;
};
PendingFwd g_pending_fwd;
using CfgC2 = ConvFwdCfg<3, 3, 2, 1, 8, 8, 8, 64, 4, 2, 2, 4, false, 1>;
using CfgC4 = ConvFwdCfg<1, 1, 2, 0, 8, 8, 8, 64, 4, 2, 2, 4, false, 1>;
}

void conv_flush_pending_fwd() {
  if (g_pending_fwd.x == nullptr) return;
  const PendingFwd p = g_pending_fwd;
  g_pending_fwd = PendingFwd{};
  run_fwd<1, 1, 2, 0, 8, 8, 8, 64, 4, 2, 2, 4, false, true>(p.x, p.w, p.y, p.B, p.g.C, p.g.Co, p.ks, p.part, p.s,
                                                           nullptr, p.defer);
}

int launch_conv_fwd(const float* x, const float* w, float* y, int B, const ConvGeom& g, float* part, hipStream_t s,
                    bool defer, double* stats_out, float* wino_u, bool pair) {
  const ConvBnStats stats{stats_out, nullptr, nullptr, nullptr, nullptr};
  const int cls = conv_direct_class(g);
  const int ks = conv_ksplit(cls, g, B, false);
  if (cls == 4 && pair && stats_out == nullptr) {
    conv_flush_pending_fwd();
    int k = ks;
    fwd_part<CfgC4>(x, w, y, part, B, g.C, g.Co, k);
    g_pending_fwd = PendingFwd{x, w, y, part, B, ks, defer, g, s};
    return (k > 1 && defer) ? k : 1;
  }
  if (cls == 2 && g_pending_fwd.x == x && g_pending_fwd.s == s && g_pending_fwd.B == B && stats_out == nullptr) {
    const PendingFwd p = g_pending_fwd;
    g_pending_fwd = PendingFwd{};
    int ka = ks, kb = p.ks;
    const FwdPart a = fwd_part<CfgC2>(x, w, y, part, B, g.C, g.Co, ka);
    const FwdPart b = fwd_part<CfgC4>(p.x, p.w, p.y, p.part, B, p.g.C, p.g.Co, kb);
    const uint3 ga = make_uint3((unsigned)(B / 4), (unsigned)(g.Co / 64), (unsigned)ka);
    const uint3 gb = make_uint3((unsigned)(B / 4), (unsigned)(p.g.Co / 64), (unsigned)kb);
    constexpr size_t lds = CfgC2::LDS_BYTES > CfgC4::LDS_BYTES ? CfgC2::LDS_BYTES : CfgC4::LDS_BYTES;
    static bool attr = false;
    if (!attr) { set_lds(ds_fwd_pair_kernel, lds); attr = true; }
    hipLaunchKernelGGL(ds_fwd_pair_kernel, dim3(ga.x * ga.y * ga.z + gb.x * gb.y * gb.z), dim3(256), lds, s, a, ga, b, gb);
    if (kb > 1 && !p.defer)
      hipLaunchKernelGGL(conv_slab_sum_kernel, dim3((unsigned)((b.slab / 4 + 15) / 16)), dim3(256), 0, s, p.part, p.y,
                         b.slab, kb, nullptr);
    if (ka > 1 && defer) return ka;
    if (ka > 1)
      hipLaunchKernelGGL(conv_slab_sum_kernel, dim3((unsigned)((a.slab / 4 + 15) / 16)), dim3(256), 0, s, part, y,
                         a.slab, ka, nullptr);
    return 1;
  }
  conv_flush_pending_fwd();
  if (wino_u != nullptr && conv_wino(cls, g, B, false)) {
    launch_wino_conv(x, wino_u, y, B, g.C, g.Co, g.H, false, 1, nullptr, ks > 1 ? ConvBnStats{} : stats, ks, part, s);
    return ks > 1 ? wino_slabs(part, y, (int64_t)B * g.Co * g.H * g.W, ks, defer, nullptr, s) : 1;
  }
  switch (cls) {
    case 0:
      return run_fwd<3, 3, 1, 1, 8, 8, 8, 64, 1, 2, 2, 4, false, true, 1, 2>(x, w, y, B, g.C, g.Co, ks, part, s,
                                                                             nullptr, defer, stats);
    case 1:
      return run_fwd<3, 3, 1, 1, 4, 4, 8, 64, 4, 2, 2, 4, false, true, 1, 2>(x, w, y, B, g.C, g.Co, ks, part, s,
                                                                             nullptr, defer);
    case 2:
      return run_fwd<3, 3, 2, 1, 8, 8, 8, 64, 4, 2, 2, 4, false, true>(x, w, y, B, g.C, g.Co, ks, part, s, nullptr,
                                                                       defer);
    case 3:
      switch (stem_psplit(B)) {
        case 4:
          return run_fwd<7, 7, 2, 3, 32, 32, 4, 64, 1, 2, 1, 7, false, false, 1, 0, 1, 4>(x, w, y, B, g.C, g.Co, 1, nullptr,
                                                                                        s, nullptr, false, stats);
        case 2:
          return run_fwd<7, 7, 2, 3, 32, 32, 4, 64, 1, 2, 1, 7, false, false, 1, 0, 1, 2>(x, w, y, B, g.C, g.Co, 1, nullptr,
                                                                                        s, nullptr, false, stats);
        default:
          return run_fwd<7, 7, 2, 3, 32, 32, 4, 64, 1, 2, 1, 7, false, false>(x, w, y, B, g.C, g.Co, 1, nullptr, s,
                                                                              nullptr, false, stats);
      }
    case 4:
      return run_fwd<1, 1, 2, 0, 8, 8, 8, 64, 4, 2, 2, 4, false, true>(x, w, y, B, g.C, g.Co, ks, part, s, nullptr,
                                                                       defer);
    case 5:
      return run_fwd<1, 1, 2, 0, 4, 4, 8, 64, 16, 2, 2, 4, false, true>(x, w, y, B, g.C, g.Co, ks, part, s, nullptr,
                                                                        defer);
    default: return 1;
  }
}

namespace {
struct PendingWgrad {
  const float* x = nullptr;
  const float* dy = nullptr;
  float* part = nullptr;
  int B = 0, imgs = 0, cls = -1;
  ConvGeom g{};
  hipStream_t s = nullptr;
};
constexpr int kPendingSlots = 2;
PendingWgrad g_pending[kPendingSlots];
unsigned g_pending_seq[kPendingSlots];
unsigned g_seq = 0;

void launch_pending(const PendingWgrad& p);
PendingWgrad* find_pending(const float* dy, int cls, int B, const ConvGeom& g, hipStream_t s) {
  for (auto& p : g_pending)
    if (p.dy == dy && p.cls == cls && p.s == s && p.B == B && p.g.C == g.C && p.g.Co == g.Co && p.g.H == g.H) return &p;
  return nullptr;
}
void flush_pending_dy(const float* dy) {
  for (auto& p : g_pending)
    if (p.dy == dy) {
      const PendingWgrad q = p;
      p = PendingWgrad{};
      launch_pending(q);
    }
}
void hold_pending(const PendingWgrad& q) {
  int k = -1;
  for (int i = 0; i < kPendingSlots; ++i)
    if (g_pending[i].dy == nullptr) { k = i; break; }
  if (k < 0) {
    k = g_pending_seq[0] <= g_pending_seq[1] ? 0 : 1;
    const PendingWgrad old = g_pending[k];
    g_pending[k] = PendingWgrad{};
    launch_pending(old);
  }
  g_pending[k] = q;
  g_pending_seq[k] = ++g_seq;
}

template <int WH, int IUPS, int R, int S, int ST, int PD, int H, int W, int CB, int BM, int NW, int NBPW, int KB>
void run_pair(const float* dy, const float* u, float* dx, int B, int inC, int outC, const float* addend,
              const ConvBnStats& st, int ks, float* part_x, const PendingWgrad& p, hipStream_t s) {
  using G = ConvWgCfg<R, S, ST, PD, H, W, CB, BM, NW, NBPW, KB>;
  auto k = wino_direct_pair_kernel<WH, IUPS, R, S, ST, PD, H, W, CB, BM, NW, NBPW, KB>;
  constexpr size_t lds = kWLds > G::LDS_BYTES ? kWLds : G::LDS_BYTES;
  static bool attr = false;
  if (!attr) { set_lds(k, lds); attr = true; }
  const WinoConvArgs a{dy, u + 16 * (int64_t)inC * outC,
                       dx, inC, outC, ks > 1 ? nullptr : addend, ks > 1 ? ConvBnStats{} : st, (inC / kWCK) / ks,
                       part_x, (int64_t)B * outC * WH * WH};
  const uint3 ga = make_uint3((unsigned)(B / wino_imgs(WH)), (unsigned)(outC / kWBM), (unsigned)ks);
  const uint3 gw = make_uint3((unsigned)(p.B / p.imgs), (unsigned)(p.g.Co / BM), (unsigned)((p.g.C + CB - 1) / CB));
  const unsigned n = ga.x * ga.y * ga.z + gw.x * gw.y * gw.z;
  hipLaunchKernelGGL(k, dim3(n), dim3(256), lds, s, a, ga, p.x, p.dy, p.part, p.g.C, p.g.Co, p.imgs, gw);
}
template <int DH, int DW, int DIMGS, int R, int S, int ST, int PD, int H, int W, int CB, int BM, int NW, int NBPW,
          int KB>
int run_direct_pair(const float* dy, const float* w, float* dx, int B, int Cin, int Kout, int ksplit, float* part,
                    const float* addend, const PendingWgrad& p, hipStream_t s) {
  using GF = ConvFwdCfg<1, 1, 1, 0, DH, DW, 8, 64, DIMGS, 2, 2, 4, true, 1>;
  using GW = ConvWgCfg<R, S, ST, PD, H, W, CB, BM, NW, NBPW, KB>;
  auto k = direct_pair_kernel<DH, DW, 64, DIMGS, R, S, ST, PD, H, W, CB, BM, NW, NBPW, KB>;
  constexpr size_t lds = GF::LDS_BYTES > GW::LDS_BYTES ? GF::LDS_BYTES : GW::LDS_BYTES;
  static bool attr = false;
  if (!attr) { set_lds(k, lds); attr = true; }
  const int nchunks = (Cin + 7) / 8;
  if (ksplit < 1 || part == nullptr) ksplit = 1;
  const int cps = (nchunks + ksplit - 1) / ksplit;
  ksplit = (nchunks + cps - 1) / cps;
  const int64_t slab = (int64_t)B * Kout * GF::PQ;
  const DirectDgradArgs a{dy, w, dx, part, Cin, Kout, cps, slab, ksplit > 1 ? nullptr : addend};
  const uint3 ga = make_uint3((unsigned)(B / DIMGS), (unsigned)(Kout / 64), (unsigned)ksplit);
  const uint3 gw = make_uint3((unsigned)(p.B / p.imgs), (unsigned)(p.g.Co / BM), (unsigned)((p.g.C + CB - 1) / CB));
  const unsigned n = ga.x * ga.y * ga.z + gw.x * gw.y * gw.z;
  hipLaunchKernelGGL(k, dim3(n), dim3(256), lds, s, a, ga, p.x, p.dy, p.part, p.g.C, p.g.Co, p.imgs, gw);
  if (ksplit > 1)
    hipLaunchKernelGGL((conv_slab_sum_ups_kernel<GF::P, GF::Q>), dim3((unsigned)((slab + 255) / 256)), dim3(256), 0, s,
                       part, dx, slab, ksplit, addend);
  return 1;
}

void launch_pending(const PendingWgrad& p) {
  if (p.cls == 0) launch_wino_wgrad(p.x, p.dy, p.part, p.B, p.g.C, p.g.Co, p.g.H, p.imgs, p.s);
  else if (p.cls == 1) run_wgrad<3, 3, 1, 1, 4, 4, 32, 32, 3, 3, 4>(p.x, p.dy, p.part, nullptr, p.B, p.g.C, p.g.Co, p.imgs, p.s);
  else if (p.cls == 2) run_wgrad<3, 3, 2, 1, 8, 8, 32, 32, 3, 3, 4>(p.x, p.dy, p.part, nullptr, p.B, p.g.C, p.g.Co, p.imgs, p.s);
  else if (p.cls == 4) run_wgrad<1, 1, 2, 0, 8, 8, 32, 32, 1, 1, 4>(p.x, p.dy, p.part, nullptr, p.B, p.g.C, p.g.Co, p.imgs, p.s);
  else run_wgrad<1, 1, 2, 0, 4, 4, 32, 32, 1, 1, 2>(p.x, p.dy, p.part, nullptr, p.B, p.g.C, p.g.Co, p.imgs, p.s);
}
}

void conv_flush_pending() {
  while (true) {
    int k = -1;
    for (int i = 0; i < kPendingSlots; ++i)
      if (g_pending[i].dy != nullptr && (k < 0 || g_pending_seq[i] < g_pending_seq[k])) k = i;
    if (k < 0) return;
    const PendingWgrad p = g_pending[k];
    g_pending[k] = PendingWgrad{};
    launch_pending(p);
  }
}

int launch_conv_dgrad(const float* dy, const float* w, float* dx, int B, const ConvGeom& g, float* part,
                      hipStream_t s, const float* addend, bool defer, const ConvBnStats* bst, float* wino_u) {
  const ConvBnStats stats = bst != nullptr ? *bst : ConvBnStats{nullptr, nullptr, nullptr, nullptr, nullptr};
  const int cls = conv_direct_class(g);
  const int ks = conv_ksplit(cls, g, B, true);
  if (wino_u != nullptr && conv_wino(cls, g, B, true)) {
    if (PendingWgrad* pp = find_pending(dy, cls, B, g, s)) {
      const PendingWgrad p = *pp;
      *pp = PendingWgrad{};
      if (cls == 0)
        launch_wino_bwd_pair(dy, wino_u, dx, B, g.Co, g.C, addend, stats, ks, part, p.x, p.part, p.imgs, s);
      else if (cls == 1)
        run_pair<4, 1, 3, 3, 1, 1, 4, 4, 32, 32, 3, 3, 4>(dy, wino_u, dx, B, g.Co, g.C, addend, stats, ks, part, p, s);
      else
        run_pair<8, 2, 3, 3, 2, 1, 8, 8, 32, 32, 3, 3, 4>(dy, wino_u, dx, B, g.Co, g.C, addend, stats, ks, part, p, s);
    } else {
      flush_pending_dy(dy);
      launch_wino_conv(dy, wino_u, dx, B, g.Co, g.C, g.H, true, cls == 2 ? 2 : 1, addend,
                       ks > 1 ? ConvBnStats{} : stats, ks, part, s);
    }
    return ks > 1 ? wino_slabs(part, dx, (int64_t)B * g.C * g.H * g.W, ks, defer, addend, s) : 1;
  }
  if (PendingWgrad* pp = (cls == 4 || cls == 5) ? find_pending(dy, cls, B, g, s) : nullptr) {
    const PendingWgrad p = *pp;
    *pp = PendingWgrad{};
    return cls == 4
        ? run_direct_pair<4, 4, 4, 1, 1, 2, 0, 8, 8, 32, 32, 1, 1, 4>(dy, w, dx, B, g.Co, g.C, ks, part, addend, p, s)
        : run_direct_pair<2, 2, 16, 1, 1, 2, 0, 4, 4, 32, 32, 1, 1, 2>(dy, w, dx, B, g.Co, g.C, ks, part, addend, p, s);
  }
  flush_pending_dy(dy);
  switch (cls) {
    case 0:
      return run_fwd<3, 3, 1, 1, 8, 8, 8, 64, 1, 2, 2, 4, true, true, 1, 2>(dy, w, dx, B, g.Co, g.C, ks, part, s,
                                                                            addend, defer, stats);
    case 1:
      return run_fwd<3, 3, 1, 1, 4, 4, 8, 64, 4, 2, 2, 4, true, true, 1, 2>(dy, w, dx, B, g.Co, g.C, ks, part, s,
                                                                            addend, defer);
    case 2:
      return run_fwd<3, 3, 1, 1, 8, 8, 8, 64, 1, 2, 2, 4, true, true, 1, 2, 2>(dy, w, dx, B, g.Co, g.C, ks, part, s,
                                                                              addend, defer, stats);
    case 4:
      return run_fwd<1, 1, 1, 0, 4, 4, 8, 64, 4, 2, 2, 4, true, true, 2>(dy, w, dx, B, g.Co, g.C, ks, part, s, addend);
    case 5:
      return run_fwd<1, 1, 1, 0, 2, 2, 8, 64, 16, 2, 2, 4, true, true, 2>(dy, w, dx, B, g.Co, g.C, ks, part, s, addend);
    default: return 1;
  }
}

void launch_conv_wgrad(const float* x, const float* dy, float* part, float* dw, int B, const ConvGeom& g,
                       hipStream_t s, bool pair) {
  const int cls = conv_direct_class(g);
  const int imgs = conv_wgrad_imgs(cls, g, B);
  if (cls == 0 && wino_wgrad_ok(g.C, g.Co, g.H)) {
    if (pair && dw == nullptr) {
      hold_pending(PendingWgrad{x, dy, part, B, imgs, cls, g, s});
      return;
    }
    launch_wino_wgrad(x, dy, part, B, g.C, g.Co, g.H, imgs, s);
    if (dw != nullptr) {
      const int64_t n = (int64_t)g.Co * g.C * 9;
      hipLaunchKernelGGL(conv_slab_sum_kernel, dim3((unsigned)((n / 4 + 15) / 16)), dim3(256), 0, s, part, dw, n,
                         B / imgs);
    }
    return;
  }
  if (pair && dw == nullptr &&
      (((cls == 1 || (cls == 2 && B <= 256)) && conv_wino(cls, g, B, true)) || cls == 4 || cls == 5)) {
    hold_pending(PendingWgrad{x, dy, part, B, imgs, cls, g, s});
    return;
  }
  switch (cls) {
    case 0: run_wgrad<3, 3, 1, 1, 8, 8, 32, 32, 3, 3, 4>(x, dy, part, dw, B, g.C, g.Co, imgs, s); break;
    case 1: run_wgrad<3, 3, 1, 1, 4, 4, 32, 32, 3, 3, 4>(x, dy, part, dw, B, g.C, g.Co, imgs, s); break;
    case 2: run_wgrad<3, 3, 2, 1, 8, 8, 32, 32, 3, 3, 4>(x, dy, part, dw, B, g.C, g.Co, imgs, s); break;
    case 3: run_wgrad<7, 7, 2, 3, 32, 32, 3, 32, 5, 1, 4>(x, dy, part, dw, B, g.C, g.Co, imgs, s); break;
    case 4: run_wgrad<1, 1, 2, 0, 8, 8, 32, 32, 1, 1, 4>(x, dy, part, dw, B, g.C, g.Co, imgs, s); break;
    case 5: run_wgrad<1, 1, 2, 0, 4, 4, 32, 32, 1, 1, 2>(x, dy, part, dw, B, g.C, g.Co, imgs, s); break;
    default: break;
  }
}

}
```

network_distributed_pytorch_amd/csrc/ndp_kernels.h:

```cpp
#pragma once
#include <hip/hip_runtime_api.h>
#include <stdint.h>

namespace ndp {

struct MatGeom {
  int32_t n, m, r;
  int32_t vec;
  int32_t p_off, q_off;
  int32_t pp_off, qp_off;
  int32_t p_chunks, q_chunks;
  int32_t pad[6];
};

struct MatPtrs {
  const float* min;
  float* e;
  const float* mread;
  float* out;
  float* mem;
  float* mom;
  float* x;
  float* g;
};

struct PItem { int32_t mat, row0, k0, k1, chunk, rb, pad[2]; };
struct QItem { int32_t mat, col0, row0, row1, chunk, cb, pad[2]; };
struct UItem { int32_t mat, row0, col0, pad; };
struct OrthItem { int32_t mat, row0, row1, wg, nwg, slab0, pad[2]; };

struct SegEntry {
  const float* src;
  float* dst;
  int64_t numel;
  int64_t stride;
  int32_t chunks;
  float div;
  int32_t vec;
  int32_t pad;
};

constexpr int kPRows = 64;
constexpr int kPK = 256;
constexpr int kPWRows = 16;
constexpr int kPKW = 1024;
constexpr int kQCols = 256;
constexpr int kQRowsMax = 256;
constexpr int kURows = 64;
constexpr int kUCols = 64;
constexpr int kUWideRows = 16;
constexpr int kUWideCols = 256;
constexpr int kUWideMaxRank = 16;
constexpr int kMaxRank = 64;
constexpr int kSegBlockElems = 2048;

struct PFin {
  float* out;
  unsigned long long* ctr;
  const SegEntry* seg;
  const int64_t* seg_prefix;
  int n_seg;
  int n_items;
};
struct QFin {
  float* out;
  unsigned long long* ctr;
  int max_chunks;
};
struct R1Step {
  const float* buf;
  float* mom;
  float* x;
  float* g;
  int64_t n;
  float div;
  int n_items;
};

void launch_psgd_p(const MatGeom* geom, const MatPtrs* ptrs, const PItem* items, int n_items,
                   const float* q_warm, float* p_part, int fuse_ef, int max_rank, hipStream_t s,
                   const float* p_prev = nullptr, PFin fin = PFin{}, int64_t n_seg_blocks = 0,
                   int item_cols = kPKW);
void launch_psgd_q(const MatGeom* geom, const MatPtrs* ptrs, const QItem* items, int n_items,
                   const float* p_hat, float* q_part, int max_rank, hipStream_t s, QFin fin = QFin{});
void launch_psgd_orth(const MatGeom* geom, const OrthItem* items, int n_items, int n_mats, float* p,
                      float p_div, float eps, int max_rank, float* partial, unsigned long long* counters,
                      unsigned* err, int n_items_total, unsigned max_spins, hipStream_t s);
int orth_rows_per_thread(int max_rank);
int orth_coresident_cap(int max_rank);
constexpr unsigned kOrthMaxSpins = 1u << 25;
void launch_psgd_update(const MatGeom* geom, const MatPtrs* ptrs, const UItem* items,
                        int n_items, const float* p_hat, const float* q_sum, float q_div,
                        float* q_warm, int mode, float lr, float momentum, int max_rank,
                        hipStream_t s, float* p_prev = nullptr, R1Step r1 = R1Step{});
void launch_rank1_step(const float* buf, float div, float* mom, float* x, float* g,
                       int64_t n, float lr, float momentum, hipStream_t s);

void launch_seg_reduce(const SegEntry* entries, const int64_t* block_prefix, int n_entries,
                       int64_t n_blocks, hipStream_t s);
void launch_sgd_momentum(float* x, const float* g, float* buf, int64_t n, float lr, float mu,
                         float div, hipStream_t s);
void launch_add(const float* a, const float* b, float* out, int64_t n, hipStream_t s);
void launch_delay_ns(int64_t ns, hipStream_t s);
void launch_flag_signal(unsigned* ctr, hipStream_t s);
void launch_flag_wait(unsigned* ctr, unsigned* seen, unsigned* err, int64_t timeout_us, hipStream_t s,
                      unsigned* host_err = nullptr);
void launch_checksum(const float* x, int64_t n, double* out, hipStream_t s);

}

namespace ndp {
int bn_slices(int N, int C, int HW);
int64_t bn_part_numel(int N, int C, int HW);
void launch_bn_fwd(const float* x, const float* res, float* y, const float* gamma, const float* beta,
                   float* rmean, float* rvar, int64_t* nbt, float* save_mean, float* save_invstd,
                   double* part, int N, int C, int HW, int S, float eps, float momentum, int relu,
                   int training, int single, hipStream_t s, const float* xpart = nullptr, int nslab = 0,
                   const double* xstats = nullptr, int xS = 0);
void launch_bn_bwd(const float* dy, const float* y, const float* x, const float* gamma, const float* save_mean,
                   const float* save_invstd, float* dx, float* dres, float* dgamma, float* dbeta, double* part,
                   int N, int C, int HW, int S, int relu, int single, hipStream_t s, const float* dypart = nullptr,
                   int nslab = 0, const float* dyadd = nullptr, const float* mbeta = nullptr,
                   const double* dstats = nullptr, int dS = 0);
bool bn_two_kernel_path(int N, int C, int HW, int single);
bool bn_pair_ok(int N, int C, int HW);
void launch_bn_pair_fwd(const float* x, const float* x2, float* y, const float* gamma, const float* beta,
                        float* rmean, float* rvar, int64_t* nbt, float* save_mean, float* save_invstd,
                        const float* gamma2, const float* beta2, float* rmean2, float* rvar2, int64_t* nbt2,
                        float* save_mean2, float* save_invstd2, int N, int C, int HW, float eps, float momentum,
                        hipStream_t s, const float* xpart, int nslab, const float* x2part, int nslab2);
void launch_bn_pair_bwd(const float* dy, const float* y, const float* x, const float* x2, const float* gamma,
                        const float* save_mean, const float* save_invstd, const float* gamma2,
                        const float* save_mean2, const float* save_invstd2, float* dx, float* dx2, float* dgamma,
                        float* dbeta, float* dgamma2, float* dbeta2, int N, int C, int HW, hipStream_t s,
                        const float* dypart, int nslab, const float* dyadd);
void bn_set_vec4(bool on);
void launch_bn_relu_maxpool(const float* x, float* y, uint8_t* idx, const float* gamma, const float* beta,
                            float* rmean, float* rvar, int64_t* nbt, float* save_mean, float* save_invstd,
                            double* part, int N, int C, int H, int W, float eps, float momentum, hipStream_t s,
                            const double* xstats = nullptr, int xS = 0);
}

namespace ndp {
int colsum_chunks(int64_t M, int N);
void launch_colsum(const float* g, int64_t M, int N, float* part, float* out, hipStream_t s);
void launch_gelu_bwd_colsum(const float* g, const float* h, float* dh, int64_t M, int N, float* part, float* out,
                            hipStream_t s);
void launch_embedding_backward(const int64_t* ids, int T, const float* gout, int V, int D, int pad, int* perm,
                               int* row_start, int* row_cnt, float* gw, hipStream_t s);
}

namespace ndp {
void launch_ce_fwd(const float* x, const int64_t* tgt, int B, int K, int64_t ignore, float* dl, float* rowloss,
                   float* loss, float* inv, unsigned* ctr, hipStream_t s, float* acc = nullptr);
void launch_ce_bwd(const float* dl, const float* g, const float* inv, float* dx, int64_t n, hipStream_t s);
}

namespace ndp {
bool ln_supported(int D);
struct LnDrop {
  const int32_t* seed;
  uint32_t thr;
  float scale;
  int mode;
  float* da;
};
void launch_ln_fwd(const float* a, const float* b, const float* gamma, const float* beta, float* y, float* s,
                   float* mean, float* rstd, int64_t R, int D, float eps, hipStream_t st, const LnDrop& dp);
int ln_bwd_wgs(int64_t R);
void launch_ln_bwd(const float* dy, const float* s, const float* mean, const float* rstd, const float* gamma,
                   float* dx, float* part, float* dgb, int64_t R, int D, hipStream_t st, const LnDrop& dp);
}

namespace ndp {
struct ConvGeom {
  int32_t C, H, W;
  int32_t Co, KH, KW;
  int32_t stride, pad;
  int32_t OH, OW;
};
void launch_toeplitz_expand(const float* w, float* wb, const ConvGeom& g, hipStream_t s);
constexpr int kMaxExpand = 24;
struct ExpandBatch {
  const float* w[kMaxExpand];
  float* wt[kMaxExpand];
  ConvGeom g[kMaxExpand];
  int64_t end[kMaxExpand];
  int n;
};
void launch_toeplitz_expand_many(const ExpandBatch& b, hipStream_t s);
struct FoldBatch {
  const float* dwt[kMaxExpand];
  float* dw[kMaxExpand];
  ConvGeom g[kMaxExpand];
  int64_t end[kMaxExpand];
  int n;
};
void launch_toeplitz_fold_many(const FoldBatch& b, hipStream_t s);
struct SlabBatch {
  const float* part[kMaxExpand];
  float* dw[kMaxExpand];
  int64_t numel[kMaxExpand];
  int slices[kMaxExpand];
  int64_t end[kMaxExpand];
  int n;
  int nt;
};
void launch_slab_sum_many(const SlabBatch& b, hipStream_t s);
void launch_gradw_finish(const SlabBatch& sb, const FoldBatch& fb, hipStream_t s);
void launch_toeplitz_fold(const float* dwb, float* dw, const ConvGeom& g, hipStream_t s);
int conv_direct_class(const ConvGeom& g);
int conv_fwd_imgs(int cls);
int conv_wgrad_imgs(int cls, const ConvGeom& g, int B);
bool conv_dgrad_direct(int cls);
int conv_ksplit(int cls, const ConvGeom& g, int B, bool dgrad);
struct ConvBnStats {
  double* out;
  const float* bx;
  const float* by;
  const float* mean;
  const float* invstd;
};
int launch_conv_fwd(const float* x, const float* w, float* y, int B, const ConvGeom& g, float* part, hipStream_t s,
                    bool defer = false, double* stats = nullptr, float* wino_u = nullptr, bool pair = false);
void conv_flush_pending_fwd();
int stem_psplit(int B);
void conv_set_stem_psplit(int p);
int conv_fwd_stats_slices(int cls, const ConvGeom& g, int B);
int launch_conv_dgrad(const float* dy, const float* w, float* dx, int B, const ConvGeom& g, float* part,
                      hipStream_t s, const float* addend = nullptr, bool defer = false,
                      const ConvBnStats* bst = nullptr, float* wino_u = nullptr);
int conv_dgrad_stats_slices(int cls, const ConvGeom& g, int B);
bool conv_wino(int cls, const ConvGeom& g, int B, bool dgrad);
bool wino_ok(int inC, int outC, int B, int H, int W, int ks);
bool wino_disabled();
void wino_set_enabled(bool on);
int wino_imgs(int H);
int64_t wino_u_numel(int inC, int outC);
void launch_wino_weights(const float* w, float* u, int Co, int C, hipStream_t s);
bool wino_wgrad_red(int B, int imgs);
bool wino_wgrad_ok(int C, int Co, int H);
void launch_wino_wgrad(const float* x, const float* dy, float* part, int B, int C, int Co, int H, int imgs,
                       hipStream_t s);
constexpr int kMaxWino = 16;
struct WinoBatch {
  const float* w[kMaxWino];
  float* u[kMaxWino];
  int Co[kMaxWino];
  int C[kMaxWino];
  int end[kMaxWino];
  int n;
};
void launch_wino_weights_many(const WinoBatch& b, hipStream_t s);
void launch_wino_conv(const float* x, const float* u, float* y, int B, int inC, int outC, int H, bool transw,
                      int iups, const float* addend, const ConvBnStats& st, int ks, float* part, hipStream_t s);
void launch_slab_sum(const float* part, float* out, int64_t n, int nslab, hipStream_t s,
                     const float* addend = nullptr);
void launch_conv_wgrad(const float* x, const float* dy, float* part, float* dw, int B, const ConvGeom& g,
                       hipStream_t s, bool pair = false);
void conv_flush_pending();
void launch_wino_bwd_pair(const float* dy, const float* u, float* dx, int B, int inC, int outC, const float* addend,
                          const ConvBnStats& st, int ks, float* part_x, const float* x, float* part_w, int imgs,
                          hipStream_t s);

struct TgIndex {
  int64_t so, si;
  int32_t sh, pad;
};
struct TgArgs {
  const float* a;
  const float* b;
  float* c;
  float* part;
  const float* addend;
  TgIndex am, ak, bk, bn, cm, cn;
  int32_t M, N, K, kchunk;
  int64_t slab;
};
constexpr int TG_POINTWISE = 0;
int tg_class(const ConvGeom& g);
TgArgs tg_args(const ConvGeom& g, int B, int dir, bool* akf, bool* bnf);
int tg_splits(const ConvGeom& g, int B, int dir);
int launch_tg_fwd(const float* x, const float* w, float* y, int B, const ConvGeom& g, float* part, hipStream_t s,
                  bool defer = false);
int launch_tg_dgrad(const float* dy, const float* w, float* dx, int B, const ConvGeom& g, float* part,
                    hipStream_t s, const float* addend = nullptr, bool defer = false);
int launch_tg_wgrad(const float* x, const float* dy, float* out, int B, const ConvGeom& g, float* part,
                    hipStream_t s, bool defer = false);
}

namespace ndp {
void launch_attn_fwd(const float* q, const float* k, const float* v, const int32_t* mask, float* o, float* lse,
                     int B, int S, int H, float scale, const int32_t* seed, float p_drop, hipStream_t s,
                     int64_t ldq = 0);
void launch_attn_bwd(const float* q, const float* k, const float* v, const int32_t* mask, const float* o,
                     const float* dout, const float* lse, float* delta, float* dq, float* dk, float* dv, int B,
                     int S, int H, float scale, const int32_t* seed, float p_drop, hipStream_t s,
                     int64_t ldq = 0);
}

namespace ndp {
struct PoolGeom {
  int32_t H, W, OH, OW;
  int32_t KH, KW, stride, pad;
};
void launch_maxpool_fwd(const float* x, float* y, uint8_t* idx, int planes, const PoolGeom& g, hipStream_t s);
struct PoolBnStats {
  const float* x;
  const float* gamma;
  const float* beta;
  const float* mean;
  const float* invstd;
  double* stats;
  int C, N;
};
bool maxpool_bwd_bnstats_ok(const PoolGeom& g);
void launch_stem_pool_bwd_apply(const float* dy, const uint8_t* idx, const float* x, const float* gamma,
                                const float* beta, const float* save_mean, const float* save_invstd,
                                const double* stats, float* dx, float* dgamma, float* dbeta, int N, int C, int H,
                                int W, hipStream_t s);
void launch_maxpool_bwd(const float* dy, const uint8_t* idx, float* dx, int planes, const PoolGeom& g,
                        hipStream_t s,
                        const PoolBnStats& bs = PoolBnStats{nullptr, nullptr, nullptr, nullptr, nullptr, nullptr, 0, 0});
}
```

network_distributed_pytorch_amd/csrc/winograd.hip:

```cpp
#include <hip/hip_runtime.h>
#include <stdlib.h>

#include <string>

#include "ndp_kernels.h"
#include "wino_dpp.h"

namespace ndp {

namespace {

template <int H, int IUPS>
__global__ __launch_bounds__(256, 2) void wino_dpp_kernel(WinoConvArgs A) {
  extern __shared__ __attribute__((aligned(16))) float smem[];
  wino_dpp_body<H, IUPS>(A, make_uint3(blockIdx.x, blockIdx.y, blockIdx.z),
                         make_uint3(gridDim.x, gridDim.y, gridDim.z), smem);
}

struct WinoWgradArgs {
  const float* x;
  const float* dy;
  float* part;
  int Cin, Cout, imgs;
};
constexpr size_t kWgRedLds = (size_t)3 * 16 * 64 * sizeof(f32x4w);
template <int H, int RED = 1>
__device__ __forceinline__ void wino_wgrad_body(const WinoWgradArgs& A, const uint3 bid, float* __restrict__ smem) {
  const float* __restrict__ x = A.x;
  const float* __restrict__ dy = A.dy;
  float* __restrict__ part = A.part;
  const int Cin = A.Cin, Cout = A.Cout;
  int imgs = A.imgs;
  constexpr int TW = H / 2, TPL = TW * TW / 4, HW = H * H;
  const int lane = threadIdx.x & 63, wave = threadIdx.x >> 6;
  const int i = lane & 15, kq = lane >> 4;
  const int blk = (int)bid.y * (4 / RED) + wave / RED, nbc = Cin / 16;
  const int cob = blk / nbc, cib = blk - cob * nbc;
  if (cob * 16 >= Cout) return;
  const int slice = bid.x;
  const int b0 = slice * imgs + (wave % RED) * (imgs / RED);
  imgs /= RED;
  const int ty = H == 8 ? kq : kq >> 1, tx0 = H == 8 ? 0 : (kq & 1);
  const float* xp = x + ((int64_t)b0 * Cin + cib * 16 + i) * HW;
  const float* gp = dy + ((int64_t)b0 * Cout + cob * 16 + i) * HW;
  float xr[2][4][H], gr[2][2][H];
  auto load = [&](int n, float (&xv)[4][H], float (&gv)[2][H]) __attribute__((always_inline)) {
    const float* xa = xp + (int64_t)n * Cin * HW;
    const float* ga = gp + (int64_t)n * Cout * HW;
#pragma unroll
    for (int r = 0; r < 4; ++r) {
      const int row = 2 * ty - 1 + r;
      const bool ok = row >= 0 && row < H;
#pragma unroll
      for (int c4 = 0; c4 < H / 4; ++c4) {
        const f32x4w v = ok ? *reinterpret_cast<const f32x4w*>(xa + row * H + 4 * c4) : f32x4w{0.f, 0.f, 0.f, 0.f};
#pragma unroll
        for (int k = 0; k < 4; ++k) xv[r][4 * c4 + k] = v[k];
      }
    }
#pragma unroll
    for (int r = 0; r < 2; ++r)
#pragma unroll
      for (int c4 = 0; c4 < H / 4; ++c4) {
        const f32x4w v = *reinterpret_cast<const f32x4w*>(ga + (2 * ty + r) * H + 4 * c4);
#pragma unroll
        for (int k = 0; k < 4; ++k) gv[r][4 * c4 + k] = v[k];
      }
  };
  f32x4w acc[16];
#pragma unroll
  for (int e = 0; e < 16; ++e) acc[e] = f32x4w{0.f, 0.f, 0.f, 0.f};
  auto step = [&](const float (&xv)[4][H], const float (&gv)[2][H]) __attribute__((always_inline)) {
#pragma unroll
    for (int s = 0; s < TPL; ++s) {
      const int tx = H == 8 ? s : tx0;
      float d[4][4];
      if constexpr (H == 8) {
#pragma unroll
        for (int r = 0; r < 4; ++r)
#pragma unroll
          for (int c = 0; c < 4; ++c) {
            const int col = 2 * s - 1 + c;
            d[r][c] = (col >= 0 && col < H) ? xv[r][col < 0 ? 0 : (col >= H ? H - 1 : col)] : 0.f;
          }
      } else {
#pragma unroll
        for (int r = 0; r < 4; ++r) {
          d[r][0] = tx ? xv[r][1] : 0.f;
          d[r][1] = tx ? xv[r][2] : xv[r][0];
          d[r][2] = tx ? xv[r][3] : xv[r][1];
          d[r][3] = tx ? 0.f : xv[r][2];
        }
      }
      float v[16], sd[4][4];
#pragma unroll
      for (int c = 0; c < 4; ++c) {
        sd[0][c] = d[0][c] - d[2][c];
        sd[1][c] = d[1][c] + d[2][c];
        sd[2][c] = d[2][c] - d[1][c];
        sd[3][c] = d[1][c] - d[3][c];
      }
#pragma unroll
      for (int r = 0; r < 4; ++r) {
        v[4 * r + 0] = sd[r][0] - sd[r][2];
        v[4 * r + 1] = sd[r][1] + sd[r][2];
        v[4 * r + 2] = sd[r][2] - sd[r][1];
        v[4 * r + 3] = sd[r][1] - sd[r][3];
      }
      float g00, g01, g10, g11;
      if constexpr (H == 8) {
        g00 = gv[0][2 * s]; g01 = gv[0][2 * s + 1]; g10 = gv[1][2 * s]; g11 = gv[1][2 * s + 1];
      } else {
        g00 = tx ? gv[0][2] : gv[0][0]; g01 = tx ? gv[0][3] : gv[0][1];
        g10 = tx ? gv[1][2] : gv[1][0]; g11 = tx ? gv[1][3] : gv[1][1];
      }
      const float t[4][2] = {{g00, g01}, {g00 + g10, g01 + g11}, {g00 - g10, g01 - g11}, {-g10, -g11}};
      float yh[16];
#pragma unroll
      for (int u = 0; u < 4; ++u) {
        yh[4 * u + 0] = t[u][0];
        yh[4 * u + 1] = t[u][0] + t[u][1];
        yh[4 * u + 2] = t[u][0] - t[u][1];
        yh[4 * u + 3] = -t[u][1];
      }
#pragma unroll
      for (int e = 0; e < 16; ++e) acc[e] = mfma16(yh[e], v[e], acc[e]);
      __builtin_amdgcn_sched_barrier(0);
    }
  };
  if constexpr (H == 4) {
    load(0, xr[0], gr[0]);
    for (int n = 0; n < imgs; n += 2) {
      if (n + 1 < imgs) load(n + 1, xr[1], gr[1]);
      step(xr[0], gr[0]);
      if (n + 1 >= imgs) break;
      if (n + 2 < imgs) load(n + 2, xr[0], gr[0]);
      step(xr[1], gr[1]);
    }
  } else {
    for (int n = 0; n < imgs; ++n) {
      load(n, xr[0], gr[0]);
      step(xr[0], gr[0]);
    }
  }
  if constexpr (RED == 4) {
    auto red = reinterpret_cast<f32x4w (*)[16][64]>(smem);
    if (wave > 0) {
#pragma unroll
      for (int e = 0; e < 16; ++e) red[wave - 1][e][lane] = acc[e];
    }
    __syncthreads();
    if (wave > 0) return;
#pragma unroll
    for (int w = 0; w < 3; ++w)
#pragma unroll
      for (int e = 0; e < 16; ++e) acc[e] += red[w][e][lane];
  } else if constexpr (RED == 2) {
    auto red = reinterpret_cast<f32x4w (*)[16][64]>(smem);
    if (wave & 1) {
#pragma unroll
      for (int e = 0; e < 16; ++e) red[wave >> 1][e][lane] = acc[e];
    }
    __syncthreads();
    if (wave & 1) return;
#pragma unroll
    for (int e = 0; e < 16; ++e) acc[e] += red[wave >> 1][e][lane];
  }
  float* out = part + (int64_t)slice * Cout * Cin * 9;
#pragma unroll
  for (int r = 0; r < 4; ++r) {
    const int co = cob * 16 + 4 * kq + r, ci = cib * 16 + i;
    float m[4][4];
#pragma unroll
    for (int e = 0; e < 16; ++e) m[e >> 2][e & 3] = acc[e][r];
    float t[3][4];
#pragma unroll
    for (int v = 0; v < 4; ++v) {
      t[0][v] = m[0][v] + 0.5f * (m[1][v] + m[2][v]);
      t[1][v] = 0.5f * (m[1][v] - m[2][v]);
      t[2][v] = 0.5f * (m[1][v] + m[2][v]) + m[3][v];
    }
    float* o = out + ((int64_t)co * Cin + ci) * 9;
#pragma unroll
    for (int a = 0; a < 3; ++a) {
      o[3 * a + 0] = t[a][0] + 0.5f * (t[a][1] + t[a][2]);
      o[3 * a + 1] = 0.5f * (t[a][1] - t[a][2]);
      o[3 * a + 2] = 0.5f * (t[a][1] + t[a][2]) + t[a][3];
    }
  }
}

template <int H, int RED = 1>
__global__ __launch_bounds__(256, 2) void wino_wgrad_kernel(WinoWgradArgs A) {
  extern __shared__ __attribute__((aligned(16))) float smem[];
  wino_wgrad_body<H, RED>(A, make_uint3(blockIdx.x, blockIdx.y, 0), smem);
}

template <int RED>
__global__ __launch_bounds__(256, 2) void wino_bwd_pair_kernel(WinoConvArgs A, uint3 ga, WinoWgradArgs W, uint3 gw) {
  extern __shared__ __attribute__((aligned(16))) float smem[];
  const unsigned na = ga.x * ga.y * ga.z;
  unsigned b = blockIdx.x;
  if (b < na) {
    const uint3 id = make_uint3(b % ga.x, (b / ga.x) % ga.y, b / (ga.x * ga.y));
    wino_dpp_body<8, 1>(A, id, ga, smem);
  } else {
    b -= na;
    wino_wgrad_body<8, RED>(W, make_uint3(b % gw.x, b / gw.x, 0), smem);
  }
}

__device__ __forceinline__ void wino_weights_block(const float* __restrict__ w, float* __restrict__ u, int Co, int C,
                                                   int uu, int blk, float (&tr)[4][16][17]) {
  const int nci = C / 16;
  const int cob = blk / nci, cib = blk - cob * nci;
  const int n = Co * C;
  {
    const int col = threadIdx.x >> 4, cil = threadIdx.x & 15;
    const int co = cob * 16 + col, ci = cib * 16 + cil;
    const float* p = w + ((int64_t)co * C + ci) * 9;
    float g[3][3];
#pragma unroll
    for (int r = 0; r < 3; ++r)
#pragma unroll
      for (int c = 0; c < 3; ++c) g[r][c] = p[3 * r + c];
    float gg[3];
#pragma unroll
    for (int c = 0; c < 3; ++c)
      gg[c] = uu == 0 ? g[0][c] : uu == 3 ? g[2][c] : 0.5f * ((g[0][c] + g[2][c]) + (uu == 1 ? g[1][c] : -g[1][c]));
    float o[4] = {gg[0], 0.5f * ((gg[0] + gg[2]) + gg[1]), 0.5f * ((gg[0] + gg[2]) - gg[1]), gg[2]};
#pragma unroll
    for (int v = 0; v < 4; ++v) {
      u[(int64_t)(4 * uu + v) * n + (int64_t)co * C + ci] = o[v];
      tr[v][cil][col] = o[v];
    }
  }
  __syncthreads();
  const int cil = threadIdx.x >> 4, col = threadIdx.x & 15;
  const int co = cob * 16 + col, ci = cib * 16 + cil;
  float* ub = u + 16 * (int64_t)n;
#pragma unroll
  for (int v = 0; v < 4; ++v) ub[(int64_t)wino_pi(4 * uu + v) * n + (int64_t)ci * Co + co] = tr[v][cil][col];
}

__global__ __launch_bounds__(256) void wino_weights_kernel(const float* __restrict__ w, float* __restrict__ u, int Co,
                                                           int C) {
  __shared__ float tr[4][16][17];
  wino_weights_block(w, u, Co, C, blockIdx.y, blockIdx.x, tr);
}

__global__ __launch_bounds__(256) void wino_weights_many_kernel(WinoBatch b) {
  __shared__ float tr[4][16][17];
  const int blk = blockIdx.x;
  int e = 0;
  while (e + 1 < b.n && blk >= b.end[e]) ++e;
  wino_weights_block(b.w[e], b.u[e], b.Co[e], b.C[e], blockIdx.y, blk - (e ? b.end[e - 1] : 0), tr);
}

}

bool wino_ok(int inC, int outC, int B, int H, int W, int ks) {
  const int wimgs = wino_imgs(H);
  return H == W && (H == 8 || H == 4) && inC % kWCK == 0 && (inC / kWCK) % ks == 0 && outC % kWBM == 0 &&
         B % wimgs == 0 && (int64_t)(B / wimgs) * (outC / kWBM) * ks >= 128 && !wino_disabled();
}
int wino_imgs(int H) { return kWImgs * (H == 4 ? 4 : 1); }
int64_t wino_u_numel(int inC, int outC) { return (int64_t)32 * inC * outC; }

static int g_wino = -1;
bool wino_disabled() {
  if (g_wino < 0) {
    const char* e = getenv("NDP_FUSION_OFF");
    const std::string s = std::string(",") + (e ? e : "") + ",";
    g_wino = (s.find(",winograd,") != std::string::npos || s.find(",all,") != std::string::npos) ? 0 : 1;
  }
  return g_wino == 0;
}
void wino_set_enabled(bool on) { g_wino = on ? 1 : 0; }

void launch_wino_weights(const float* w, float* u, int Co, int C, hipStream_t s) {
  hipLaunchKernelGGL(wino_weights_kernel, dim3((unsigned)((Co / 16) * (C / 16)), 4), dim3(256), 0, s, w, u, Co, C);
}

void launch_wino_weights_many(const WinoBatch& b, hipStream_t s) {
  if (b.n <= 0) return;
  hipLaunchKernelGGL(wino_weights_many_kernel, dim3((unsigned)b.end[b.n - 1], 4), dim3(256), 0, s, b);
}

template <int H, int IUPS>
static void run_wino(const float* x, const float* u, float* y, int B, int inC, int outC, const float* addend,
                     const ConvBnStats& st, int ks, float* part, hipStream_t s) {
  static bool attr = false;
  if (!attr) {
    hipFuncSetAttribute(reinterpret_cast<const void*>(wino_dpp_kernel<H, IUPS>),
                        hipFuncAttributeMaxDynamicSharedMemorySize, (int)kWLds);
    attr = true;
  }
  const int64_t slab = (int64_t)B * outC * H * H;
  const WinoConvArgs a{x, u, y, inC, outC, ks > 1 ? nullptr : addend, st, (inC / kWCK) / ks, part, slab};
  hipLaunchKernelGGL((wino_dpp_kernel<H, IUPS>),
                     dim3((unsigned)(B / wino_imgs(H)), (unsigned)(outC / kWBM), (unsigned)ks), dim3(256), kWLds, s, a);
}

void launch_wino_conv(const float* x, const float* u, float* y, int B, int inC, int outC, int H, bool transw,
                      int iups, const float* addend, const ConvBnStats& st, int ks, float* part, hipStream_t s) {
  const float* uk = transw ? u + 16 * (int64_t)inC * outC : u;
  if (H == 4) run_wino<4, 1>(x, uk, y, B, inC, outC, addend, st, ks, part, s);
  else if (iups == 2) run_wino<8, 2>(x, uk, y, B, inC, outC, addend, st, ks, part, s);
  else run_wino<8, 1>(x, uk, y, B, inC, outC, addend, st, ks, part, s);
}

bool wino_wgrad_ok(int C, int Co, int H) { return H == 8 && C % 16 == 0 && Co % 16 == 0 && !wino_disabled(); }
bool wino_wgrad_red(int B, int imgs) { return imgs % 4 == 0 && (B <= 128 || (B >= 256 && imgs == 16)); }
static int wgrad_red(int B, int C, int Co, int imgs) {
  if (wino_wgrad_red(B, imgs)) return 4;
  return (B >= 512 && imgs % 2 == 0 && ((Co / 16) * (C / 16)) % 2 == 0) ? 2 : 1;
}
void launch_wino_wgrad(const float* x, const float* dy, float* part, int B, int C, int Co, int H, int imgs,
                       hipStream_t s) {
  if (H != 8) return;
  const WinoWgradArgs a{x, dy, part, C, Co, imgs};
  const int red = wgrad_red(B, C, Co, imgs);
  if (red == 4) {
    const dim3 grid((unsigned)(B / imgs), (unsigned)((Co / 16) * (C / 16)));
    hipLaunchKernelGGL((wino_wgrad_kernel<8, 4>), grid, dim3(256), kWgRedLds, s, a);
  } else if (red == 2) {
    const dim3 grid((unsigned)(B / imgs), (unsigned)((Co / 16) * (C / 16) / 2));
    hipLaunchKernelGGL((wino_wgrad_kernel<8, 2>), grid, dim3(256), kWgRedLds, s, a);
  } else {
    const dim3 grid((unsigned)(B / imgs), (unsigned)(((Co / 16) * (C / 16) + 3) / 4));
    hipLaunchKernelGGL((wino_wgrad_kernel<8, 1>), grid, dim3(256), 0, s, a);
  }
}

void launch_wino_bwd_pair(const float* dy, const float* u, float* dx, int B, int inC, int outC, const float* addend,
                          const ConvBnStats& st, int ks, float* part_x, const float* x, float* part_w, int imgs,
                          hipStream_t s) {
  const float* uk = u + 16 * (int64_t)inC * outC;
  const WinoConvArgs a{dy, uk, dx, inC, outC, ks > 1 ? nullptr : addend, ks > 1 ? ConvBnStats{} : st, (inC / kWCK) / ks,
                       part_x, (int64_t)B * outC * 64};
  const uint3 ga = make_uint3((unsigned)(B / wino_imgs(8)), (unsigned)(outC / kWBM), (unsigned)ks);
  const WinoWgradArgs w{x, dy, part_w, outC, inC, imgs};
  const int C = outC, Co = inC;
  const int red = wgrad_red(B, C, Co, imgs);
  const int nb = (Co / 16) * (C / 16);
  const uint3 gw = make_uint3((unsigned)(B / imgs), (unsigned)(red == 4 ? nb : red == 2 ? nb / 2 : (nb + 3) / 4), 1);
  const unsigned n = ga.x * ga.y * ga.z + gw.x * gw.y;
  const size_t lds = kWLds > kWgRedLds ? kWLds : kWgRedLds;
  static bool attr = false;
  if (!attr) {
    hipFuncSetAttribute(reinterpret_cast<const void*>(wino_bwd_pair_kernel<4>), hipFuncAttributeMaxDynamicSharedMemorySize,
                        (int)lds);
    hipFuncSetAttribute(reinterpret_cast<const void*>(wino_bwd_pair_kernel<1>), hipFuncAttributeMaxDynamicSharedMemorySize,
                        (int)lds);
    hipFuncSetAttribute(reinterpret_cast<const void*>(wino_bwd_pair_kernel<2>), hipFuncAttributeMaxDynamicSharedMemorySize,
                        (int)lds);
    attr = true;
  }
  if (red == 4) hipLaunchKernelGGL(wino_bwd_pair_kernel<4>, dim3(n), dim3(256), lds, s, a, ga, w, gw);
  else if (red == 2) hipLaunchKernelGGL(wino_bwd_pair_kernel<2>, dim3(n), dim3(256), lds, s, a, ga, w, gw);
  else hipLaunchKernelGGL(wino_bwd_pair_kernel<1>, dim3(n), dim3(256), lds, s, a, ga, w, gw);
}

}
```

network_distributed_pytorch_amd/knobs.py:

```python
from __future__ import annotations

import os

__all__ = ["FUSIONS", "fusion_on"]

FUSIONS = {
    "slab_links": "split-K conv slabs summed by the neighbouring BN kernel (models/resnet.py, ops/slablink.py)",
    "branch_links": "downsample-block grad-x of conv1 + 1x1 downsample shared in place (ops/gradlink.py)",
    "conv_bnstats": "BN forward statistics from the direct-conv epilogue (ops/conv.py)",
    "bn_bwd_stats": "BN backward statistics from the grad-x epilogue / pool backward (ops/batchnorm.py)",
    "bn_vec4": "float4 single-launch small-map BN kernel (csrc/batchnorm.hip; off: the scalar one)",
    "winograd": "F(2x2,3x3) Winograd for the layer1 3x3 forward / grad-x (csrc/winograd.hip)",
    "wino_pair": "a conv's grad-x and grad-W in one launch (csrc/winograd.hip, csrc/conv.hip pairs)",
    "ds_fwd_pair": "a downsample block's conv1 and 1x1 downsample forward in one launch (csrc/conv.hip)",
    "stem_pool": "stem BN -> ReLU -> max-pool in one pass (ops/batchnorm.py)",
    "stem_bwd": "stem max-pool backward + BN backward apply from the pooled gradient in one pass (ops/batchnorm.py)",
    "bn_pair": "downsample block's bn2 + downsample BN + ReLU in one launch per direction (ops/batchnorm.py)",
    "defer_gradw": "grad-W slab sums / folds batched at the end of backward (ops/gradfinish.py)",
    "grad_arena": "dense-arm gradients written straight into the bucket arena (ops/gradarena.py)",
    "tgemm": "strided / tabled MFMA GEMM convs for 1x1 layers (ops/tgconv.py)",
    "tuned_gemms": "hipBLASLt algorithm table for the Toeplitz GEMMs (ops/gemm_tuning.py)",
    "lazy_ef": "PowerSGD error feedback formed in the next P pass (parallel/powersgd.py)",
    "psgd_fin": "PowerSGD P / Q split-K sums, rank-1 pack and rank-1 step inside the P / Q / update launches",
    "defer_uploads": "capture-safe table uploads batched per graph (utils/graph.py)",
    "fused_ce": "native softmax cross-entropy (ops/loss.py)",
    "fused_ln": "native residual add + LayerNorm (+ dropout) (ops/layernorm.py)",
    "ln_links": "DistilBERT residual gradients folded into the sublayer GEMMs (models/distilbert.py)",
    "packed_qkv": "one QKV projection GEMM over the three weights in place (models/distilbert.py)",
    "fused_gelu": "native GELU backward + bias column sums (ops/linear.py)",
}

_OFF = {t.strip() for t in os.environ.get("NDP_FUSION_OFF", "").split(",") if t.strip()}
_unknown = _OFF - set(FUSIONS) - {"all"}
if _unknown:
    raise ValueError(f"NDP_FUSION_OFF: unknown fusion(s) {sorted(_unknown)}; known: {sorted(FUSIONS)}")


def fusion_on(name: str) -> bool:
    if name not in FUSIONS:
        raise KeyError(name)
    return "all" not in _OFF and name not in _OFF
```

Baseline: 372,300 samples/s.

## Pipeline grad-W operands: LDS prefetch in Winograd wgrad, multi-image stages in direct wgrad

Adds a prefetch path to the layer1 Winograd grad-W kernel that issues global-to-LDS loads (global_load_lds) for the next image while the current one is computed. The layer2 direct grad-W kernel now loads and stores several images (4) per double-buffered stage, which cuts the number of barriers and store phases per slice. Both paths are on by default behind a new wgrad_pipe fusion knob. In exchange the kernels use more LDS and registers, which may lower occupancy.

New measurement: 377,500 samples/s (median of 6 runs). 1.01x the previous value.

```diff
diff --git a/network_distributed_pytorch_amd/csrc/bindings.cpp b/network_distributed_pytorch_amd/csrc/bindings.cpp
--- a/network_distributed_pytorch_amd/csrc/bindings.cpp
+++ b/network_distributed_pytorch_amd/csrc/bindings.cpp
@@ -1386,6 +1386,12 @@
   m.def("bn_pair_bwd", &bn_pair_bwd);
   m.def("wino_set_enabled", &ndp::wino_set_enabled);
   m.def("conv_set_stem_psplit", &ndp::conv_set_stem_psplit);
+  m.def("conv_set_wgrad_stage", [](int n) {
+    TORCH_CHECK(ndp::conv_set_wgrad_stage(n), "conv_set_wgrad_stage: 0 (auto), 1 or 4 images per stage; ", n,
+                " is not built");
+  });
+  m.def("conv_pair_launches", &ndp::conv_pair_launches);
+  m.def("wino_set_wgrad_prefetch", &ndp::wino_set_wgrad_prefetch);
   m.def("bn_slices", &bn_slices);
   m.def("slab_sum", &slab_sum);
   m.def("bn_part_numel", &bn_part_numel);
diff --git a/network_distributed_pytorch_amd/csrc/conv.hip b/network_distributed_pytorch_amd/csrc/conv.hip
--- a/network_distributed_pytorch_amd/csrc/conv.hip
+++ b/network_distributed_pytorch_amd/csrc/conv.hip
@@ -1,5 +1,7 @@
 #include <hip/hip_runtime.h>
 #include <stdlib.h>
+
+#include <string>
 
 #include "ndp_kernels.h"
 #include "wino_dpp.h"
@@ -751,23 +753,24 @@
   static constexpr size_t MAIN_BYTES = 2 * (size_t)(A_SZ + B_SZ) * sizeof(float);
   static constexpr size_t EPI_BYTES = TAPMAJ ? (size_t)BM * LDJ * sizeof(float) : 0;
   static constexpr size_t LDS_BYTES = MAIN_BYTES > EPI_BYTES ? MAIN_BYTES : EPI_BYTES;
+  static constexpr size_t lds_bytes(int ips) { return ips * MAIN_BYTES > EPI_BYTES ? ips * MAIN_BYTES : EPI_BYTES; }
   static_assert(MB * JB == NW * NBPW, "every wave owns NBPW 32x32 blocks");
   static_assert(P % 2 == 0 && PQ % 4 == 0 && HW % 4 == 0 && NSTEP % KB == 0, "pixel pairing / float4 loads");
 };
 
-template <int R, int S, int ST, int PD, int H, int W, int CB, int BM, int NW, int NBPW, int KB>
+template <int R, int S, int ST, int PD, int H, int W, int CB, int BM, int NW, int NBPW, int KB, int IPS = 1>
 __device__ __forceinline__ void conv_wgrad_body(const float* __restrict__ x, const float* __restrict__ dy,
                                                 float* __restrict__ part, int Cin, int Kout, int imgs_per_slice,
                                                 const uint3 bid, float* __restrict__ smem) {
   using G = ConvWgCfg<R, S, ST, PD, H, W, CB, BM, NW, NBPW, KB>;
   float* As = smem;
-  float* Bs = smem + 2 * G::A_SZ;
+  float* Bs = smem + 2 * IPS * G::A_SZ;
   const int tid = threadIdx.x, lane = tid & 63, wave = tid >> 6;
   const int h = lane >> 5, l32 = lane & 31;
   const int slice = bid.x, m0 = bid.y * BM, c0 = bid.z * CB;
   const int bb = slice * imgs_per_slice;
 
-  for (int i = tid; i < 2 * G::B_SZ; i += G::NT) Bs[i] = 0.f;
+  for (int i = tid; i < 2 * IPS * G::B_SZ; i += G::NT) Bs[i] = 0.f;
 
   int a_base[NBPW], b_base[NBPW];
 #pragma unroll
@@ -782,48 +785,54 @@
     b_base[t] = (j < G::J) ? c * G::HWp + r * G::Wp + s + h * (G::P / 2) * ST * G::Wp : 0;
   }
 
-  f32x4c ra[G::A_PER_T], rb[G::B_PER_T];
+  f32x4c ra[IPS][G::A_PER_T], rb[IPS][G::B_PER_T];
   auto load = [&](int b) {
 #pragma unroll
-    for (int i = 0; i < G::A_PER_T; ++i) {
-      const int e = tid + G::NT * i;
-      f32x4c v = {0.f, 0.f, 0.f, 0.f};
-      if (e < G::A4) v = *reinterpret_cast<const f32x4c*>(dy + ((int64_t)b * Kout + m0) * G::PQ + 4 * e);
-      ra[i] = v;
-    }
-#pragma unroll
-    for (int i = 0; i < G::B_PER_T; ++i) {
-      const int e = tid + G::NT * i;
-      f32x4c v = {0.f, 0.f, 0.f, 0.f};
-      if (e < G::B4 && c0 + (4 * e) / G::HW < Cin)
-        v = *reinterpret_cast<const f32x4c*>(x + ((int64_t)b * Cin + c0) * G::HW + 4 * e);
-      rb[i] = v;
+    for (int ii = 0; ii < IPS; ++ii) {
+#pragma unroll
+      for (int i = 0; i < G::A_PER_T; ++i) {
+        const int e = tid + G::NT * i;
+        f32x4c v = {0.f, 0.f, 0.f, 0.f};
+        if (e < G::A4) v = *reinterpret_cast<const f32x4c*>(dy + ((int64_t)(b + ii) * Kout + m0) * G::PQ + 4 * e);
+        ra[ii][i] = v;
+      }
+#pragma unroll
+      for (int i = 0; i < G::B_PER_T; ++i) {
+        const int e = tid + G::NT * i;
+        f32x4c v = {0.f, 0.f, 0.f, 0.f};
+        if (e < G::B4 && c0 + (4 * e) / G::HW < Cin)
+          v = *reinterpret_cast<const f32x4c*>(x + ((int64_t)(b + ii) * Cin + c0) * G::HW + 4 * e);
+        rb[ii][i] = v;
+      }
     }
   };
   auto store = [&](int buf) {
-    float* A = As + buf * G::A_SZ;
-    float* B = Bs + buf * G::B_SZ;
-#pragma unroll
-    for (int i = 0; i < G::A_PER_T; ++i) {
-      const int e = tid + G::NT * i;
-      if (e < G::A4) {
-        const int m = (4 * e) / G::PQ, pq = 4 * e - m * G::PQ;
-        float* d = A + m * G::LDY + pq;
-        if constexpr (G::AVW) {
-          *reinterpret_cast<f32x4c*>(d) = ra[i];
-        } else {
-          d[0] = ra[i].x; d[1] = ra[i].y; d[2] = ra[i].z; d[3] = ra[i].w;
-        }
-      }
-    }
-#pragma unroll
-    for (int i = 0; i < G::B_PER_T; ++i) {
-      const int e = tid + G::NT * i;
-      if (e < G::B4) {
-        const int c = (4 * e) / G::HW, hw = 4 * e - c * G::HW;
-        const int hh = hw / W, ww = hw - hh * W;
-        float* d = B + c * G::HWp + (hh + PD) * G::Wp + ww + PD;
-        d[0] = rb[i].x; d[1] = rb[i].y; d[2] = rb[i].z; d[3] = rb[i].w;
+#pragma unroll
+    for (int ii = 0; ii < IPS; ++ii) {
+      float* A = As + (buf * IPS + ii) * G::A_SZ;
+      float* B = Bs + (buf * IPS + ii) * G::B_SZ;
+#pragma unroll
+      for (int i = 0; i < G::A_PER_T; ++i) {
+        const int e = tid + G::NT * i;
+        if (e < G::A4) {
+          const int m = (4 * e) / G::PQ, pq = 4 * e - m * G::PQ;
+          float* d = A + m * G::LDY + pq;
+          if constexpr (G::AVW) {
+            *reinterpret_cast<f32x4c*>(d) = ra[ii][i];
+          } else {
+            d[0] = ra[ii][i].x; d[1] = ra[ii][i].y; d[2] = ra[ii][i].z; d[3] = ra[ii][i].w;
+          }
+        }
+      }
+#pragma unroll
+      for (int i = 0; i < G::B_PER_T; ++i) {
+        const int e = tid + G::NT * i;
+        if (e < G::B4) {
+          const int c = (4 * e) / G::HW, hw = 4 * e - c * G::HW;
+          const int hh = hw / W, ww = hw - hh * W;
+          float* d = B + c * G::HWp + (hh + PD) * G::Wp + ww + PD;
+          d[0] = rb[ii][i].x; d[1] = rb[ii][i].y; d[2] = rb[ii][i].z; d[3] = rb[ii][i].w;
+        }
       }
     }
   };
@@ -838,44 +847,48 @@
   __syncthreads();
   store(0);
   __syncthreads();
-  for (int i = 0; i < imgs_per_slice; ++i) {
+  const int stages = imgs_per_slice / IPS;
+  for (int i = 0; i < stages; ++i) {
     const int cur = i & 1;
-    if (i + 1 < imgs_per_slice) load(bb + i + 1);
-    const float* A = As + cur * G::A_SZ;
-    const float* B = Bs + cur * G::B_SZ;
-    float av[2][KB][NBPW], bv[2][KB][NBPW];
-    auto fetch = [&](int blk, int slot) {
-#pragma unroll
-      for (int k = 0; k < KB; ++k) {
-        const int t = blk * KB + k;
-        const int p = t / G::Q, q = t - p * G::Q;
-#pragma unroll
-        for (int u = 0; u < NBPW; ++u) {
-          if constexpr (!G::AVW) av[slot][k][u] = A[a_base[u] + t];
-          bv[slot][k][u] = B[b_base[u] + p * ST * G::Wp + q * ST];
-        }
-      }
-      if constexpr (G::AVW) {
-#pragma unroll
-        for (int u = 0; u < NBPW; ++u)
-#pragma unroll
-          for (int q4 = 0; q4 < KB / 4; ++q4) {
-            const f32x4c v = *reinterpret_cast<const f32x4c*>(A + a_base[u] + blk * KB + 4 * q4);
-#pragma unroll
-            for (int j = 0; j < 4; ++j) av[slot][4 * q4 + j][u] = v[j];
+    if (i + 1 < stages) load(bb + (i + 1) * IPS);
+#pragma unroll
+    for (int ii = 0; ii < IPS; ++ii) {
+      const float* A = As + (cur * IPS + ii) * G::A_SZ;
+      const float* B = Bs + (cur * IPS + ii) * G::B_SZ;
+      float av[2][KB][NBPW], bv[2][KB][NBPW];
+      auto fetch = [&](int blk, int slot) {
+#pragma unroll
+        for (int k = 0; k < KB; ++k) {
+          const int t = blk * KB + k;
+          const int p = t / G::Q, q = t - p * G::Q;
+#pragma unroll
+          for (int u = 0; u < NBPW; ++u) {
+            if constexpr (!G::AVW) av[slot][k][u] = A[a_base[u] + t];
+            bv[slot][k][u] = B[b_base[u] + p * ST * G::Wp + q * ST];
           }
-      }
-    };
-    fetch(0, 0);
-#pragma unroll
-    for (int blk = 0; blk < G::NBLK; ++blk) {
-      if (blk + 1 < G::NBLK) fetch(blk + 1, (blk + 1) & 1);
-#pragma unroll
-      for (int k = 0; k < KB; ++k)
-#pragma unroll
-        for (int u = 0; u < NBPW; ++u) acc[u] = mfma32(av[blk & 1][k][u], bv[blk & 1][k][u], acc[u]);
-    }
-    if (i + 1 < imgs_per_slice) store(cur ^ 1);
+        }
+        if constexpr (G::AVW) {
+#pragma unroll
+          for (int u = 0; u < NBPW; ++u)
+#pragma unroll
+            for (int q4 = 0; q4 < KB / 4; ++q4) {
+              const f32x4c v = *reinterpret_cast<const f32x4c*>(A + a_base[u] + blk * KB + 4 * q4);
+#pragma unroll
+              for (int j = 0; j < 4; ++j) av[slot][4 * q4 + j][u] = v[j];
+            }
+        }
+      };
+      fetch(0, 0);
+#pragma unroll
+      for (int blk = 0; blk < G::NBLK; ++blk) {
+        if (blk + 1 < G::NBLK) fetch(blk + 1, (blk + 1) & 1);
+#pragma unroll
+        for (int k = 0; k < KB; ++k)
+#pragma unroll
+          for (int u = 0; u < NBPW; ++u) acc[u] = mfma32(av[blk & 1][k][u], bv[blk & 1][k][u], acc[u]);
+      }
+    }
+    if (i + 1 < stages) store(cur ^ 1);
     __syncthreads();
   }
 
@@ -930,16 +943,17 @@
   }
 }
 
-template <int R, int S, int ST, int PD, int H, int W, int CB, int BM, int NW, int NBPW, int KB>
+template <int R, int S, int ST, int PD, int H, int W, int CB, int BM, int NW, int NBPW, int KB, int IPS = 1>
 __global__ __launch_bounds__(64 * NW) void conv_wgrad_kernel(const float* __restrict__ x, const float* __restrict__ dy,
                                                              float* __restrict__ part, int Cin, int Kout,
                                                              int imgs_per_slice) {
   extern __shared__ __attribute__((aligned(16))) float smem[];
-  conv_wgrad_body<R, S, ST, PD, H, W, CB, BM, NW, NBPW, KB>(x, dy, part, Cin, Kout, imgs_per_slice,
-                                                           make_uint3(blockIdx.x, blockIdx.y, blockIdx.z), smem);
-}
-
-template <int WH, int IUPS, int R, int S, int ST, int PD, int H, int W, int CB, int BM, int NW, int NBPW, int KB>
+  conv_wgrad_body<R, S, ST, PD, H, W, CB, BM, NW, NBPW, KB, IPS>(x, dy, part, Cin, Kout, imgs_per_slice,
+                                                                make_uint3(blockIdx.x, blockIdx.y, blockIdx.z), smem);
+}
+
+template <int WH, int IUPS, int R, int S, int ST, int PD, int H, int W, int CB, int BM, int NW, int NBPW, int KB,
+          int IPS = 1>
 __global__ __launch_bounds__(256, 2) void wino_direct_pair_kernel(WinoConvArgs A, uint3 ga, const float* __restrict__ x,
                                                                   const float* __restrict__ dy, float* __restrict__ part,
                                                                   int Cin, int Kout, int imgs, uint3 gw) {
@@ -952,7 +966,7 @@
   } else {
     if (threadIdx.x >= 64 * NW) return;
     b -= na;
-    conv_wgrad_body<R, S, ST, PD, H, W, CB, BM, NW, NBPW, KB>(
+    conv_wgrad_body<R, S, ST, PD, H, W, CB, BM, NW, NBPW, KB, IPS>(
         x, dy, part, Cin, Kout, imgs, make_uint3(b % gw.x, (b / gw.x) % gw.y, b / (gw.x * gw.y)), smem);
   }
 }
@@ -1163,19 +1177,39 @@
                      addend);
 }
 
-template <int R, int S, int ST, int PD, int H, int W, int CB, int BM, int NW, int NBPW, int KB>
+constexpr int kWgIps = 4;
+static int g_wgrad_stage = 0;
+bool conv_set_wgrad_stage(int n) {
+  if (n != 0 && n != 1 && n != kWgIps) return false;
+  g_wgrad_stage = n;
+  return true;
+}
+static int64_t g_pair_launches = 0;
+int64_t conv_pair_launches() { return g_pair_launches; }
+static bool wgrad_staged(int imgs) {
+  const bool on = g_wgrad_stage ? g_wgrad_stage == kWgIps : !wgrad_pipe_off();
+  return on && imgs % kWgIps == 0 && imgs >= 2 * kWgIps;
+}
+
+template <int R, int S, int ST, int PD, int H, int W, int CB, int BM, int NW, int NBPW, int KB, int IPS = 1>
 static void run_wgrad(const float* x, const float* dy, float* part, float* dw, int B, int Cin, int Kout,
                       int imgs, hipStream_t s) {
   using G = ConvWgCfg<R, S, ST, PD, H, W, CB, BM, NW, NBPW, KB>;
-  auto k = conv_wgrad_kernel<R, S, ST, PD, H, W, CB, BM, NW, NBPW, KB>;
+  auto k = conv_wgrad_kernel<R, S, ST, PD, H, W, CB, BM, NW, NBPW, KB, IPS>;
+  constexpr size_t lds = G::lds_bytes(IPS);
   static bool attr = false;
-  if (!attr) { set_lds(k, G::LDS_BYTES); attr = true; }
+  if (!attr) { set_lds(k, lds); attr = true; }
   const int slices = B / imgs;
-  hipLaunchKernelGGL(k, dim3(slices, Kout / BM, (Cin + CB - 1) / CB), dim3(G::NT), G::LDS_BYTES, s, x, dy, part, Cin,
+  hipLaunchKernelGGL(k, dim3(slices, Kout / BM, (Cin + CB - 1) / CB), dim3(G::NT), lds, s, x, dy, part, Cin,
                      Kout, imgs);
   if (dw == nullptr) return;
   const int64_t n = (int64_t)Kout * Cin * G::RS;
   hipLaunchKernelGGL(conv_slab_sum_kernel, dim3((unsigned)((n / 4 + 15) / 16)), dim3(256), 0, s, part, dw, n, slices);
+}
+static void run_wgrad_c1(const float* x, const float* dy, float* part, float* dw, int B, int Cin, int Kout, int imgs,
+                         hipStream_t s) {
+  if (wgrad_staged(imgs)) run_wgrad<3, 3, 1, 1, 4, 4, 32, 32, 3, 3, 4, kWgIps>(x, dy, part, dw, B, Cin, Kout, imgs, s);
+  else run_wgrad<3, 3, 1, 1, 4, 4, 32, 32, 3, 3, 4>(x, dy, part, dw, B, Cin, Kout, imgs, s);
 }
 
 int conv_direct_class(const ConvGeom& g) {
@@ -1412,12 +1446,13 @@
   g_pending_seq[k] = ++g_seq;
 }
 
-template <int WH, int IUPS, int R, int S, int ST, int PD, int H, int W, int CB, int BM, int NW, int NBPW, int KB>
+template <int WH, int IUPS, int R, int S, int ST, int PD, int H, int W, int CB, int BM, int NW, int NBPW, int KB,
+          int IPS = 1>
 void run_pair(const float* dy, const float* u, float* dx, int B, int inC, int outC, const float* addend,
               const ConvBnStats& st, int ks, float* part_x, const PendingWgrad& p, hipStream_t s) {
   using G = ConvWgCfg<R, S, ST, PD, H, W, CB, BM, NW, NBPW, KB>;
-  auto k = wino_direct_pair_kernel<WH, IUPS, R, S, ST, PD, H, W, CB, BM, NW, NBPW, KB>;
-  constexpr size_t lds = kWLds > G::LDS_BYTES ? kWLds : G::LDS_BYTES;
+  auto k = wino_direct_pair_kernel<WH, IUPS, R, S, ST, PD, H, W, CB, BM, NW, NBPW, KB, IPS>;
+  constexpr size_t lds = kWLds > G::lds_bytes(IPS) ? kWLds : G::lds_bytes(IPS);
   static bool attr = false;
   if (!attr) { set_lds(k, lds); attr = true; }
   const WinoConvArgs a{dy, u + 16 * (int64_t)inC * outC,
@@ -1427,6 +1462,7 @@
   const uint3 gw = make_uint3((unsigned)(p.B / p.imgs), (unsigned)(p.g.Co / BM), (unsigned)((p.g.C + CB - 1) / CB));
   const unsigned n = ga.x * ga.y * ga.z + gw.x * gw.y * gw.z;
   hipLaunchKernelGGL(k, dim3(n), dim3(256), lds, s, a, ga, p.x, p.dy, p.part, p.g.C, p.g.Co, p.imgs, gw);
+  ++g_pair_launches;
 }
 template <int DH, int DW, int DIMGS, int R, int S, int ST, int PD, int H, int W, int CB, int BM, int NW, int NBPW,
           int KB>
@@ -1448,6 +1484,7 @@
   const uint3 gw = make_uint3((unsigned)(p.B / p.imgs), (unsigned)(p.g.Co / BM), (unsigned)((p.g.C + CB - 1) / CB));
   const unsigned n = ga.x * ga.y * ga.z + gw.x * gw.y * gw.z;
   hipLaunchKernelGGL(k, dim3(n), dim3(256), lds, s, a, ga, p.x, p.dy, p.part, p.g.C, p.g.Co, p.imgs, gw);
+  ++g_pair_launches;
   if (ksplit > 1)
     hipLaunchKernelGGL((conv_slab_sum_ups_kernel<GF::P, GF::Q>), dim3((unsigned)((slab + 255) / 256)), dim3(256), 0, s,
                        part, dx, slab, ksplit, addend);
@@ -1456,7 +1493,7 @@
 
 void launch_pending(const PendingWgrad& p) {
   if (p.cls == 0) launch_wino_wgrad(p.x, p.dy, p.part, p.B, p.g.C, p.g.Co, p.g.H, p.imgs, p.s);
-  else if (p.cls == 1) run_wgrad<3, 3, 1, 1, 4, 4, 32, 32, 3, 3, 4>(p.x, p.dy, p.part, nullptr, p.B, p.g.C, p.g.Co, p.imgs, p.s);
+  else if (p.cls == 1) run_wgrad_c1(p.x, p.dy, p.part, nullptr, p.B, p.g.C, p.g.Co, p.imgs, p.s);
   else if (p.cls == 2) run_wgrad<3, 3, 2, 1, 8, 8, 32, 32, 3, 3, 4>(p.x, p.dy, p.part, nullptr, p.B, p.g.C, p.g.Co, p.imgs, p.s);
   else if (p.cls == 4) run_wgrad<1, 1, 2, 0, 8, 8, 32, 32, 1, 1, 4>(p.x, p.dy, p.part, nullptr, p.B, p.g.C, p.g.Co, p.imgs, p.s);
   else run_wgrad<1, 1, 2, 0, 4, 4, 32, 32, 1, 1, 2>(p.x, p.dy, p.part, nullptr, p.B, p.g.C, p.g.Co, p.imgs, p.s);
@@ -1484,8 +1521,12 @@
     if (PendingWgrad* pp = find_pending(dy, cls, B, g, s)) {
       const PendingWgrad p = *pp;
       *pp = PendingWgrad{};
-      if (cls == 0)
+      if (cls == 0) {
         launch_wino_bwd_pair(dy, wino_u, dx, B, g.Co, g.C, addend, stats, ks, part, p.x, p.part, p.imgs, s);
+        ++g_pair_launches;
+      } else if (cls == 1 && wgrad_staged(p.imgs))
+        run_pair<4, 1, 3, 3, 1, 1, 4, 4, 32, 32, 3, 3, 4, kWgIps>(dy, wino_u, dx, B, g.Co, g.C, addend, stats, ks, part, p,
+                                                                  s);
       else if (cls == 1)
         run_pair<4, 1, 3, 3, 1, 1, 4, 4, 32, 32, 3, 3, 4>(dy, wino_u, dx, B, g.Co, g.C, addend, stats, ks, part, p, s);
       else
@@ -1547,7 +1588,7 @@
   }
   switch (cls) {
     case 0: run_wgrad<3, 3, 1, 1, 8, 8, 32, 32, 3, 3, 4>(x, dy, part, dw, B, g.C, g.Co, imgs, s); break;
-    case 1: run_wgrad<3, 3, 1, 1, 4, 4, 32, 32, 3, 3, 4>(x, dy, part, dw, B, g.C, g.Co, imgs, s); break;
+    case 1: run_wgrad_c1(x, dy, part, dw, B, g.C, g.Co, imgs, s); break;
     case 2: run_wgrad<3, 3, 2, 1, 8, 8, 32, 32, 3, 3, 4>(x, dy, part, dw, B, g.C, g.Co, imgs, s); break;
     case 3: run_wgrad<7, 7, 2, 3, 32, 32, 3, 32, 5, 1, 4>(x, dy, part, dw, B, g.C, g.Co, imgs, s); break;
     case 4: run_wgrad<1, 1, 2, 0, 8, 8, 32, 32, 1, 1, 4>(x, dy, part, dw, B, g.C, g.Co, imgs, s); break;
diff --git a/network_distributed_pytorch_amd/csrc/ndp_kernels.h b/network_distributed_pytorch_amd/csrc/ndp_kernels.h
--- a/network_distributed_pytorch_amd/csrc/ndp_kernels.h
+++ b/network_distributed_pytorch_amd/csrc/ndp_kernels.h
@@ -242,6 +242,10 @@
 bool wino_wgrad_ok(int C, int Co, int H);
 void launch_wino_wgrad(const float* x, const float* dy, float* part, int B, int C, int Co, int H, int imgs,
                        hipStream_t s);
+bool wgrad_pipe_off();
+void wino_set_wgrad_prefetch(bool on);
+bool conv_set_wgrad_stage(int n);
+int64_t conv_pair_launches();
 constexpr int kMaxWino = 16;
 struct WinoBatch {
   const float* w[kMaxWino];
diff --git a/network_distributed_pytorch_amd/csrc/winograd.hip b/network_distributed_pytorch_amd/csrc/winograd.hip
--- a/network_distributed_pytorch_amd/csrc/winograd.hip
+++ b/network_distributed_pytorch_amd/csrc/winograd.hip
@@ -24,8 +24,13 @@
   int Cin, Cout, imgs;
 };
 constexpr size_t kWgRedLds = (size_t)3 * 16 * 64 * sizeof(f32x4w);
-template <int H, int RED = 1>
+constexpr int kWgZone = 2 * 16 * 64;
+static_assert((size_t)4 * kWgZone * sizeof(float) <= kWgRedLds, "landing zones fit the RED buffer");
+#define NDP_WG_GLOBAL __attribute__((address_space(1)))
+#define NDP_WG_LDS __attribute__((address_space(3)))
+template <int H, int RED = 1, bool PF = false>
 __device__ __forceinline__ void wino_wgrad_body(const WinoWgradArgs& A, const uint3 bid, float* __restrict__ smem) {
+  static_assert(!PF || H == 8, "the LDS landing zone is laid out for the 8x8 maps");
   const float* __restrict__ x = A.x;
   const float* __restrict__ dy = A.dy;
   float* __restrict__ part = A.part;
@@ -67,6 +72,48 @@
         for (int k = 0; k < 4; ++k) gv[r][4 * c4 + k] = v[k];
       }
   };
+  float* zone = smem + wave * kWgZone;
+  const int pch = lane >> 4, pck = ((lane & 15) ^ pch) * 4;
+  auto issue = [&](int n) __attribute__((always_inline)) {
+    if constexpr (PF) {
+      const float* xa = x + ((int64_t)(b0 + n) * Cin + cib * 16) * HW;
+      const float* ga = dy + ((int64_t)(b0 + n) * Cout + cob * 16) * HW;
+#pragma unroll
+      for (int j = 0; j < 4; ++j) {
+        const int off = (4 * j + pch) * HW + (pck ^ (16 * j));
+        __builtin_amdgcn_global_load_lds((const NDP_WG_GLOBAL void*)(xa + off), (NDP_WG_LDS void*)(zone + j * 256), 16,
+                                         0, 0);
+        __builtin_amdgcn_global_load_lds((const NDP_WG_GLOBAL void*)(ga + off),
+                                         (NDP_WG_LDS void*)(zone + 16 * HW + j * 256), 16, 0, 0);
+      }
+    }
+  };
+  auto land = [&](float (&xv)[4][H], float (&gv)[2][H]) __attribute__((always_inline)) {
+    if constexpr (PF) {
+      const float* zx = zone + i * HW;
+      const float* zg = zone + 16 * HW + i * HW;
+#pragma unroll
+      for (int r = 0; r < 4; ++r) {
+        const int row = 2 * ty - 1 + r;
+        const bool ok = row >= 0 && row < H;
+        const int rc = row < 0 ? 0 : (row >= H ? H - 1 : row);
+#pragma unroll
+        for (int c4 = 0; c4 < H / 4; ++c4) {
+          const f32x4w v = *reinterpret_cast<const f32x4w*>(zx + 4 * ((2 * rc + c4) ^ i));
+#pragma unroll
+          for (int k = 0; k < 4; ++k) xv[r][4 * c4 + k] = ok ? v[k] : 0.f;
+        }
+      }
+#pragma unroll
+      for (int r = 0; r < 2; ++r)
+#pragma unroll
+        for (int c4 = 0; c4 < H / 4; ++c4) {
+          const f32x4w v = *reinterpret_cast<const f32x4w*>(zg + 4 * ((2 * (2 * ty + r) + c4) ^ i));
+#pragma unroll
+          for (int k = 0; k < 4; ++k) gv[r][4 * c4 + k] = v[k];
+        }
+    }
+  };
   f32x4w acc[16];
 #pragma unroll
   for (int e = 0; e < 16; ++e) acc[e] = f32x4w{0.f, 0.f, 0.f, 0.f};
@@ -137,6 +184,18 @@
       if (n + 2 < imgs) load(n + 2, xr[0], gr[0]);
       step(xr[1], gr[1]);
     }
+  } else if constexpr (PF) {
+    issue(0);
+    for (int n = 0; n < imgs; ++n) {
+      asm volatile("s_waitcnt vmcnt(0)" ::: "memory");
+      land(xr[0], gr[0]);
+      asm volatile("s_waitcnt lgkmcnt(0)" ::: "memory");
+      __builtin_amdgcn_sched_barrier(0);
+      if (n + 1 < imgs) issue(n + 1);
+      __builtin_amdgcn_sched_barrier(0);
+      step(xr[0], gr[0]);
+    }
+    if constexpr (RED > 1) __syncthreads();
   } else {
     for (int n = 0; n < imgs; ++n) {
       load(n, xr[0], gr[0]);
@@ -190,13 +249,13 @@
   }
 }
 
-template <int H, int RED = 1>
+template <int H, int RED = 1, bool PF = false>
 __global__ __launch_bounds__(256, 2) void wino_wgrad_kernel(WinoWgradArgs A) {
   extern __shared__ __attribute__((aligned(16))) float smem[];
-  wino_wgrad_body<H, RED>(A, make_uint3(blockIdx.x, blockIdx.y, 0), smem);
-}
-
-template <int RED>
+  wino_wgrad_body<H, RED, PF>(A, make_uint3(blockIdx.x, blockIdx.y, 0), smem);
+}
+
+template <int RED, bool PF = false>
 __global__ __launch_bounds__(256, 2) void wino_bwd_pair_kernel(WinoConvArgs A, uint3 ga, WinoWgradArgs W, uint3 gw) {
   extern __shared__ __attribute__((aligned(16))) float smem[];
   const unsigned na = ga.x * ga.y * ga.z;
@@ -206,7 +265,7 @@
     wino_dpp_body<8, 1>(A, id, ga, smem);
   } else {
     b -= na;
-    wino_wgrad_body<8, RED>(W, make_uint3(b % gw.x, b / gw.x, 0), smem);
+    wino_wgrad_body<8, RED, PF>(W, make_uint3(b % gw.x, b / gw.x, 0), smem);
   }
 }
 
@@ -277,6 +336,14 @@
   return g_wino == 0;
 }
 void wino_set_enabled(bool on) { g_wino = on ? 1 : 0; }
+bool wgrad_pipe_off() {
+  static const bool off = [] {
+    const char* e = getenv("NDP_FUSION_OFF");
+    const std::string s = std::string(",") + (e ? e : "") + ",";
+    return s.find(",wgrad_pipe,") != std::string::npos || s.find(",all,") != std::string::npos;
+  }();
+  return off;
+}
 
 void launch_wino_weights(const float* w, float* u, int Co, int C, hipStream_t s) {
   hipLaunchKernelGGL(wino_weights_kernel, dim3((unsigned)((Co / 16) * (C / 16)), 4), dim3(256), 0, s, w, u, Co, C);
@@ -316,21 +383,38 @@
   if (wino_wgrad_red(B, imgs)) return 4;
   return (B >= 512 && imgs % 2 == 0 && ((Co / 16) * (C / 16)) % 2 == 0) ? 2 : 1;
 }
+static int g_wgrad_pf = -1;
+static bool wgrad_prefetch(int imgs, int red) {
+  return (g_wgrad_pf < 0 ? !wgrad_pipe_off() : g_wgrad_pf == 1) && imgs / red >= 2;
+}
+void wino_set_wgrad_prefetch(bool on) { g_wgrad_pf = on ? 1 : 0; }
+
+template <int RED, bool PF>
+static void run_wino_wgrad(const WinoWgradArgs& a, int B, int nb, hipStream_t s) {
+  const dim3 grid((unsigned)(B / a.imgs), (unsigned)((nb + 4 / RED - 1) / (4 / RED)));
+  hipLaunchKernelGGL((wino_wgrad_kernel<8, RED, PF>), grid, dim3(256), (RED > 1 || PF) ? kWgRedLds : 0, s, a);
+}
 void launch_wino_wgrad(const float* x, const float* dy, float* part, int B, int C, int Co, int H, int imgs,
                        hipStream_t s) {
   if (H != 8) return;
   const WinoWgradArgs a{x, dy, part, C, Co, imgs};
-  const int red = wgrad_red(B, C, Co, imgs);
-  if (red == 4) {
-    const dim3 grid((unsigned)(B / imgs), (unsigned)((Co / 16) * (C / 16)));
-    hipLaunchKernelGGL((wino_wgrad_kernel<8, 4>), grid, dim3(256), kWgRedLds, s, a);
-  } else if (red == 2) {
-    const dim3 grid((unsigned)(B / imgs), (unsigned)((Co / 16) * (C / 16) / 2));
-    hipLaunchKernelGGL((wino_wgrad_kernel<8, 2>), grid, dim3(256), kWgRedLds, s, a);
-  } else {
-    const dim3 grid((unsigned)(B / imgs), (unsigned)(((Co / 16) * (C / 16) + 3) / 4));
-    hipLaunchKernelGGL((wino_wgrad_kernel<8, 1>), grid, dim3(256), 0, s, a);
-  }
+  const int red = wgrad_red(B, C, Co, imgs), nb = (Co / 16) * (C / 16);
+  const bool pf = wgrad_prefetch(imgs, red);
+  if (red == 4) pf ? run_wino_wgrad<4, true>(a, B, nb, s) : run_wino_wgrad<4, false>(a, B, nb, s);
+  else if (red == 2) pf ? run_wino_wgrad<2, true>(a, B, nb, s) : run_wino_wgrad<2, false>(a, B, nb, s);
+  else pf ? run_wino_wgrad<1, true>(a, B, nb, s) : run_wino_wgrad<1, false>(a, B, nb, s);
+}
+
+template <int RED, bool PF>
+static void run_wino_pair(unsigned n, size_t lds, hipStream_t s, const WinoConvArgs& a, uint3 ga,
+                          const WinoWgradArgs& w, uint3 gw) {
+  static bool attr = false;
+  if (!attr) {
+    hipFuncSetAttribute(reinterpret_cast<const void*>(wino_bwd_pair_kernel<RED, PF>),
+                        hipFuncAttributeMaxDynamicSharedMemorySize, (int)lds);
+    attr = true;
+  }
+  hipLaunchKernelGGL((wino_bwd_pair_kernel<RED, PF>), dim3(n), dim3(256), lds, s, a, ga, w, gw);
 }
 
 void launch_wino_bwd_pair(const float* dy, const float* u, float* dx, int B, int inC, int outC, const float* addend,
@@ -347,19 +431,11 @@
   const uint3 gw = make_uint3((unsigned)(B / imgs), (unsigned)(red == 4 ? nb : red == 2 ? nb / 2 : (nb + 3) / 4), 1);
   const unsigned n = ga.x * ga.y * ga.z + gw.x * gw.y;
   const size_t lds = kWLds > kWgRedLds ? kWLds : kWgRedLds;
-  static bool attr = false;
-  if (!attr) {
-    hipFuncSetAttribute(reinterpret_cast<const void*>(wino_bwd_pair_kernel<4>), hipFuncAttributeMaxDynamicSharedMemorySize,
-                        (int)lds);
-    hipFuncSetAttribute(reinterpret_cast<const void*>(wino_bwd_pair_kernel<1>), hipFuncAttributeMaxDynamicSharedMemorySize,
-                        (int)lds);
-    hipFuncSetAttribute(reinterpret_cast<const void*>(wino_bwd_pair_kernel<2>), hipFuncAttributeMaxDynamicSharedMemorySize,
-                        (int)lds);
-    attr = true;
-  }
-  if (red == 4) hipLaunchKernelGGL(wino_bwd_pair_kernel<4>, dim3(n), dim3(256), lds, s, a, ga, w, gw);
-  else if (red == 2) hipLaunchKernelGGL(wino_bwd_pair_kernel<2>, dim3(n), dim3(256), lds, s, a, ga, w, gw);
-  else hipLaunchKernelGGL(wino_bwd_pair_kernel<1>, dim3(n), dim3(256), lds, s, a, ga, w, gw);
-}
-
-}
+  const bool pf = wgrad_prefetch(imgs, red);
+  if (red == 4) pf ? run_wino_pair<4, true>(n, lds, s, a, ga, w, gw) : run_wino_pair<4, false>(n, lds, s, a, ga, w, gw);
+  else if (red == 2)
+    pf ? run_wino_pair<2, true>(n, lds, s, a, ga, w, gw) : run_wino_pair<2, false>(n, lds, s, a, ga, w, gw);
+  else pf ? run_wino_pair<1, true>(n, lds, s, a, ga, w, gw) : run_wino_pair<1, false>(n, lds, s, a, ga, w, gw);
+}
+
+}
diff --git a/network_distributed_pytorch_amd/knobs.py b/network_distributed_pytorch_amd/knobs.py
--- a/network_distributed_pytorch_amd/knobs.py
+++ b/network_distributed_pytorch_amd/knobs.py
@@ -12,6 +12,8 @@
     "bn_vec4": "float4 single-launch small-map BN kernel (csrc/batchnorm.hip; off: the scalar one)",
     "winograd": "F(2x2,3x3) Winograd for the layer1 3x3 forward / grad-x (csrc/winograd.hip)",
     "wino_pair": "a conv's grad-x and grad-W in one launch (csrc/winograd.hip, csrc/conv.hip pairs)",
+    "wgrad_pipe": "grad-W operand pipelining: LDS prefetch of the next image in the layer1 Winograd grad-W, several "
+                  "images per stage in the layer2 direct grad-W (csrc/winograd.hip, csrc/conv.hip)",
     "ds_fwd_pair": "a downsample block's conv1 and 1x1 downsample forward in one launch (csrc/conv.hip)",
     "stem_pool": "stem BN -> ReLU -> max-pool in one pass (ops/batchnorm.py)",
     "stem_bwd": "stem max-pool backward + BN backward apply from the pooled gradient in one pass (ops/batchnorm.py)",
```
